# aitrailblazer/VectorRAGQuantization

Measured on AMD Instinct MI355X. Metric: queries/sec + recall@10 vs float32, d=1024 3-phase search at 1/2/4/8 GPUs, higher is better.
Workload: dtype u8+f64; 1 GPU; BASELINE config 4: CohereEnhancedVectorDB 3-phase search, row-sharded over N GPUs + RCCL all_gather of per-shard top-K, 100000000 x 1024 corpus, nq=1024 queries per step; corpus_rows=100000000, rows_per_gpu=100000000, nq=1024, k=10, binary_oversample=10, int8_oversample=3, parallelism=1 GPU

## Files before the change

### vectorragquantization_amd/csrc/hamming_mfma.hip

```cpp
#include <stdlib.h>

#include "mfma_common.h"
#include "mfma_fp4.h"
#include "mfma_hits.h"
#include "vrq_internal.h"
#include "vrq_scan.h"

namespace vrq {

constexpr int KS = 16;
constexpr int NG = 2 * KS;
constexpr int PKT = RT * 128;
constexpr int NPK = 4;
constexpr int NUB = 3;
constexpr int UBT = NG * 1024;
constexpr int GPW = (PKT / 1024) / MWAVES;
constexpr int BAHEAD = 3;
constexpr int NRING = BAHEAD < 4 ? 4 : 8;
#ifndef VRQ_K1M_NSR
#define VRQ_K1M_NSR 4
#endif
#ifndef VRQ_K1M_DMA_SHADOW
#define VRQ_K1M_DMA_SHADOW 1
#endif
template <int MB>
struct MfmaShape {
  static constexpr int QPW = 32 * MB;
  static constexpr int QPB = MWAVES * QPW;
  static constexpr int NSR = VRQ_K1M_NSR < MB ? VRQ_K1M_NSR : MB;
  static constexpr int SMEM =
      NPK * PKT + NUB * UBT + NUB * RT * 4 + MWAVES * QPW * 8 + MWAVES * (STG + 1) * 4 + MWAVES * MB * 128;
  static_assert(SMEM <= 160 * 1024, "LDS budget");
};
constexpr int kMbLarge = 4, kMbSmall = 2;
constexpr int kMbLargeMinQueries = 512;
constexpr int kRowsMaxQueries = 128;

__device__ __forceinline__ int pk_slot(int r, int c) { return r * 8 + (c ^ ((r >> 1) & 7)); }

constexpr int ENT_V_BIAS = 1025;


constexpr int k1m_pre(int g) { return ((g & 7) == 1 ? 1 : 0) + (g == 12 ? 2 : 0); }
constexpr int k1m_post(int g, int mb, int nsr, bool dense) {
  const int j = g & 15;
  return ((g & 7) == 6 ? 2 : 0) + (g == 28 ? 1 : 0) + (!dense && j >= 4 + mb + nsr && j < 4 + 2 * mb ? 4 : 0) +
         (!dense && g == 20 + mb ? 1 : 0) + (!dense && g == 24 + mb ? 1 : 0);
}
constexpr int k1m_wait(int gi, int mb, int nsr, bool dense) {
  const int g0 = gi - BAHEAD;
  int n = 1 + k1m_pre(gi);
  for (int g = g0 < 0 ? 0 : g0; g < gi; ++g) n += (g == g0 ? 0 : 1) + k1m_pre(g) + k1m_post(g, mb, nsr, dense);
  return n < 15 ? n : 15;
}

template <int MODE, int MB>
__global__ __launch_bounds__(MWAVES * 64, 1) void hamming_mfma_kernel(
    const uint8_t* __restrict__ codes, int64_t n, int64_t row_begin, const uint8_t* __restrict__ queries, int nq,
    const int32_t* __restrict__ tau, uint64_t* __restrict__ cand, int32_t* __restrict__ ccnt, int capc,
    int64_t chunk_rows, int64_t chunk_stride, int64_t tile_stride, int nchunks, int nqb,
    const int32_t* __restrict__ rerun,
    const int32_t* __restrict__ qbflag, uint16_t* __restrict__ dv, int64_t dv_stride) {
  constexpr bool DENSE = MODE == MFMA_SAMPLE;
  constexpr int QPW = MfmaShape<MB>::QPW, QPB = MfmaShape<MB>::QPB;
  constexpr int NSR = DENSE ? 0 : MfmaShape<MB>::NSR;
  __shared__ __attribute__((aligned(16))) uint8_t smem[MfmaShape<MB>::SMEM];
  uint8_t* pk = smem;
  uint8_t* ub = smem + NPK * PKT;
  int32_t* pcr = (int32_t*)(smem + NPK * PKT + NUB * UBT);
  const int w = __builtin_amdgcn_readfirstlane(threadIdx.x >> 6);
  int32_t* lcnt = pcr + NUB * RT + w * QPW;
  int32_t* tq = pcr + NUB * RT + MWAVES * QPW + w * QPW;
  int32_t* stg = pcr + NUB * RT + 2 * MWAVES * QPW + w * (STG + 1);

  const int l = lane_id();
  const int h = l >> 5, ri = l & 31;
  const int nb = gridDim.x, b = blockIdx.x;
  const int xcd = b & 7, slot = b >> 3, q8 = nb >> 3, r8 = nb & 7;
  const int L = (xcd < r8 ? xcd * (q8 + 1) : r8 * (q8 + 1) + (xcd - r8) * q8) + slot;
  const int chunk = L / nqb;
  const int qb = L - chunk * nqb;
  if (chunk >= nchunks) return;
  if (qbflag && qbflag[qb] == 0) return;
#ifdef VRQ_K1M_STAMPS
  const uint64_t st_start = __builtin_amdgcn_s_memrealtime();
#endif
  const int64_t row0 = row_begin + (int64_t)chunk * chunk_stride;
  const bool strided = tile_stride != RT;
  const int64_t row1 = strided ? n : (row0 + chunk_rows < n) ? row0 + chunk_rows : n;
  if (row0 >= row1) return;
  const int nrows = strided ? (int)chunk_rows : (int)(row1 - row0);
  const int ntiles = (nrows + RT - 1) / RT;

  static_assert(GPW == 2, "piece offsets derived for two pieces per wave");
  uint32_t doff0;
  {
    const int p = w * GPW * 64 + l;
    const int r = p >> 3, c = (p & 7) ^ ((r >> 1) & 7);
    doff0 = (uint32_t)(r * 128 + c * 16);
  }
  auto issue = [&](int t) __attribute__((always_inline)) {
    uint8_t* buf = pk + (t % NPK) * PKT;
    const int64_t tr0 = row0 + (int64_t)t * tile_stride;
    uint32_t d0 = doff0;
    asm volatile("" : "+v"(d0));
    const uint32_t doff[GPW] = {d0, (d0 + 1024u) ^ 64u};
    if (__builtin_expect(tr0 + RT <= row1, 1)) {
      const uint8_t* base = codes + tr0 * 128;
#pragma unroll
      for (int i = 0; i < GPW; ++i)
        __builtin_amdgcn_global_load_lds(base + doff[i], (__attribute__((address_space(3))) void*)(buf + (w * GPW + i) * 1024),
                                         16, 0, 0);
    } else {
#pragma unroll
      for (int i = 0; i < GPW; ++i) {
        int64_t row = tr0 + (doff[i] >> 7);
        row = row < row1 ? row : row1 - 1;
        __builtin_amdgcn_global_load_lds(codes + row * 128 + (doff[i] & 127),
                                         (__attribute__((address_space(3))) void*)(buf + (w * GPW + i) * 1024), 16, 0, 0);
      }
    }
  };
  auto issue_piece = [&](const uint8_t* base, uint32_t slot_off, auto I) __attribute__((always_inline)) {
    constexpr int i = decltype(I)::value;
    uint32_t d0 = doff0;
    asm volatile("" : "+v"(d0));
    const uint32_t d = i == 0 ? d0 : (d0 + 1024u) ^ 64u;
    __builtin_amdgcn_global_load_lds(base + d, (__attribute__((address_space(3))) void*)(pk + slot_off + (w * GPW + i) * 1024),
                                     16, 0, 0);
  };
  const uint32_t pk0 = lds_addr(pk), ub0 = lds_addr(ub), pcr0 = lds_addr(pcr);
  const uint32_t lc0 = lds_addr(lcnt), stg0 = lds_addr(stg);
  uint32_t usrc[4], udst[4];
#pragma unroll
  for (int u = 0; u < 4; ++u) {
    const int unit = 4 * w + u, nblk = unit >> 3, p = unit & 7;
    const int r = nblk * 32 + ri;
    usrc[u] = (uint32_t)(pk_slot(r, p) * 16 + h * 8);
    udst[u] = (uint32_t)(((nblk * KS + 2 * p) * 64 + l) * 16);
  }
  const int pr = 16 * w + (l >> 2), pc0 = 2 * (l & 3);
  const uint32_t psrc0 = (uint32_t)(pk_slot(pr, pc0) * 16), psrc1 = (uint32_t)(pk_slot(pr, pc0 + 1) * 16);
  auto unpack_write = [&](const v2i& v, int u, uint32_t ubuf) __attribute__((always_inline)) {
    lds_write128(ubuf + udst[u], unpack_row32((uint32_t)v.x));
    lds_write128(ubuf + udst[u] + 1024, unpack_row32((uint32_t)v.y));
  };
  auto rowpc_write = [&](const v4i& a, const v4i& c, uint32_t pbuf) __attribute__((always_inline)) {
    int pc = (__popc(a.x) + __popc(a.y) + __popc(a.z) + __popc(a.w)) +
             (__popc(c.x) + __popc(c.y) + __popc(c.z) + __popc(c.w));
    pc += __builtin_amdgcn_update_dpp(0, pc, 0xB1, 0xf, 0xf, false);
    pc += __builtin_amdgcn_update_dpp(0, pc, 0x4E, 0xf, 0xf, false);
    if ((l & 3) == 0) lds_write32(pbuf + (uint32_t)(pr * 4), pc);
  };

  for (int t = 0; t < NPK && t < ntiles; ++t) issue(t);

  const int qbase = qb * QPB + w * QPW;
  v4i A[MB][KS];
#pragma unroll
  for (int m = 0; m < MB; ++m) {
    const int q = qbase + 32 * m + ri;
    const bool qok = q < nq && (!rerun || rerun[q]);
    const uint4* qp = reinterpret_cast<const uint4*>(queries + (int64_t)(qok ? q : 0) * 128);
    int pc = 0;
#pragma unroll
    for (int c = 0; c < 8; ++c) {
      const uint4 v = qp[c];
      const uint32_t wd[4] = {qok ? v.x : 0u, qok ? v.y : 0u, qok ? v.z : 0u, qok ? v.w : 0u};
      pc += __popc(wd[0]) + __popc(wd[1]) + __popc(wd[2]) + __popc(wd[3]);
      A[m][2 * c] = unpack_query32(h ? wd[2] : wd[0]);
      A[m][2 * c + 1] = unpack_query32(h ? wd[3] : wd[1]);
    }
    if (h == 0) tq[32 * m + ri] = DENSE ? 0 : qok ? tau[q] - pc : -0x40000000;
  }
#pragma unroll
  for (int m = 0; m < MB; ++m)
#pragma unroll
    for (int s = 0; s < KS; ++s) asm volatile("" : "+a"(A[m][s]));
  float* sd = reinterpret_cast<float*>(pcr + NUB * RT + 2 * MWAVES * QPW + MWAVES * (STG + 1)) + w * MB * 32;
#pragma unroll
  for (int m = 0; m < MB; ++m)
    if (l < 32) {
      const int g = l & 15, hh = l >> 4;
      sd[m * 32 + l] = 0.5f * (float)tq[32 * m + (g & 3) + 8 * (g >> 2) + 4 * hh];
    }
  const uint32_t sd0 = lds_addr(sd) + (uint32_t)(h * 64);
  auto load_seed = [&](v16f& a, int m) __attribute__((always_inline)) {
    v4i p0, p1, p2, p3;
    lds_read128(p0, sd0 + (uint32_t)(m * 128));
    lds_read128(p1, sd0 + (uint32_t)(m * 128 + 16));
    lds_read128(p2, sd0 + (uint32_t)(m * 128 + 32));
    lds_read128(p3, sd0 + (uint32_t)(m * 128 + 48));
    const v16i x = __builtin_shufflevector(__builtin_shufflevector(p0, p1, 0, 1, 2, 3, 4, 5, 6, 7),
                                           __builtin_shufflevector(p2, p3, 0, 1, 2, 3, 4, 5, 6, 7), 0, 1, 2, 3, 4,
                                           5, 6, 7, 8, 9, 10, 11, 12, 13, 14, 15);
    a = __builtin_bit_cast(v16f, x);
  };
  for (int i = l; i < QPW; i += 64) lcnt[i] = 0;
  __syncthreads();
  auto wait_tiles = [&](int k) __attribute__((always_inline)) {
    if (k <= 0) wait_vm<0>();
    else if (k == 1) wait_vm<GPW>();
    else if (k == 2) wait_vm<2 * GPW>();
    else if (k == 3) wait_vm<3 * GPW>();
    else wait_vm<4 * GPW>();
  };
  static_assert(NPK - 2 <= 4, "wait_tiles covers up to 4 tiles in flight");
  const int nissued = ntiles < NPK ? ntiles : NPK;
  wait_tiles(nissued - 2);
  barrier_all();
  {
    v2i pv[8];
    v4i pa[2], pb[2];
#pragma unroll
    for (int t = 0; t < 2; ++t) {
#pragma unroll
      for (int u = 0; u < 4; ++u) lds_read64(pv[4 * t + u], pk0 + (uint32_t)(t * PKT) + usrc[u]);
      lds_read128(pa[t], pk0 + (uint32_t)(t * PKT) + psrc0);
      lds_read128(pb[t], pk0 + (uint32_t)(t * PKT) + psrc1);
    }
    asm volatile("s_waitcnt lgkmcnt(0)"
                 : "+v"(pv[0]), "+v"(pv[1]), "+v"(pv[2]), "+v"(pv[3]), "+v"(pv[4]), "+v"(pv[5]), "+v"(pv[6]),
                   "+v"(pv[7]), "+v"(pa[0]), "+v"(pa[1]), "+v"(pb[0]), "+v"(pb[1])::"memory");
#pragma unroll
    for (int t = 0; t < 2; ++t) {
#pragma unroll
      for (int u = 0; u < 4; ++u) unpack_write(pv[4 * t + u], u, ub0 + (uint32_t)(t * UBT));
      rowpc_write(pa[t], pb[t], pcr0 + (uint32_t)(t * RT * 4));
    }
  }
  wait_tiles(nissued - 3);
  wait_lgkm0();

  const int64_t qstride = (int64_t)nchunks * capc;
  uint64_t* const cbase = cand + ((int64_t)qbase * nchunks + chunk) * capc;
  int nst = 0;
  int fe = 0, fpos = 0, nfl = 0;
  auto fkey = [&](int e, int64_t base_row) __attribute__((always_inline)) {
    return ((uint64_t)(uint32_t)(e >> ENT_V_SHIFT) << KEY_ROW_BITS) | (uint64_t)(base_row + (e & 127));
  };
  auto store_flushed = [&](int t) __attribute__((always_inline)) {
    if (__builtin_expect(nfl != 0, 0)) {
      const int ql = (fe >> ENT_Q_SHIFT) & 127;
#ifndef VRQ_K1M_PROBE_NOSTORE
      if (l < nfl && fpos < capc) cbase[ql * qstride + fpos] = fkey(fe, row0 + (int64_t)(t - 2) * RT);
#endif
      nfl = 0;
    }
  };
  auto flush_from = [&](int i_begin, int64_t base_row) __attribute__((always_inline)) {
    int lf = l;
    asm volatile("" : "+v"(lf));
    if (nst > STG) {
      for (int i = lf; i < QPW; i += 64) lds_add32(lc0 + (uint32_t)(i * 4), capc + 1);
      nst = STG;
    }
    for (int i0 = i_begin; i0 < nst; i0 += 64) {
      const int i = i0 + lf;
      int e = 0, pos = 0;
      if (i < nst) lds_read32(e, stg0 + (uint32_t)(i * 4));
      asm volatile("s_waitcnt lgkmcnt(0)" : "+v"(e)::"memory");
      const int ql = (e >> ENT_Q_SHIFT) & 127;
      if (i < nst) lds_add_rtn32(pos, lc0 + (uint32_t)(ql * 4), 1);
      asm volatile("s_waitcnt lgkmcnt(0)" : "+v"(pos)::"memory");
      if (i < nst && pos < capc) cbase[ql * qstride + pos] = fkey(e, base_row);
    }
    nst = 0;
  };
  auto block_hits = [&](const v16f& a, int m, int pc, float hp, int rel7) __attribute__((always_inline)) {
#pragma unroll
    for (int g = 0; g < 16; ++g) {
      const uint64_t mask = __ballot(a[g] > hp);
      if (mask) {
        int lo = l;
        asm volatile("" : "+v"(lo));
        if ((mask >> lo) & 1) {
          const int below = __builtin_amdgcn_mbcnt_hi((uint32_t)(mask >> 32),
                                                      __builtin_amdgcn_mbcnt_lo((uint32_t)mask, 0));
          const int ql = 32 * m + (g & 3) + 8 * (g >> 2) + 4 * (lo >> 5);
          const int v = pc - (int)(2.0f * a[g]);
          const int pos = nst + below < STG ? nst + below : STG;
          lds_write32(stg0 + (uint32_t)(pos * 4), ((v + ENT_V_BIAS) << ENT_V_SHIFT) | (ql << ENT_Q_SHIFT) | (rel7 - ri + (lo & 31)));
        }
        nst += __popcll(mask);
      }
    }
  };
  auto block_hits_fast = [&](const v16f& a, int m, int pc, float hp, int rel7) __attribute__((always_inline)) {
    uint32_t m16 = 0, mmid = 0, mhi = 0;
#pragma unroll
    for (int g = 0; g < 7; ++g) m16 |= (a[g] > hp ? 1u : 0u) << g;
    asm volatile("" : "+v"(m16));
    VRQ_SCHED_FENCE();
#pragma unroll
    for (int g = 7; g < 14; ++g) mmid |= (a[g] > hp ? 1u : 0u) << (g - 7);
    asm volatile("" : "+v"(mmid));
    VRQ_SCHED_FENCE();
#pragma unroll
    for (int g = 14; g < 16; ++g) mhi |= (a[g] > hp ? 1u : 0u) << (g - 14);
    asm volatile("" : "+v"(mmid), "+v"(mhi));
    m16 |= (mmid << 7) | (mhi << 14);
#ifdef VRQ_K1M_PROBE_NOSLOW
    if (false) {
#else
    if (__ballot((m16 & (m16 - 1)) != 0)) {
#endif
      block_hits(a, m, pc, hp, rel7);
    } else {
      const uint64_t lanes = __ballot(m16 != 0);
      if (m16) {
        const v16i b = __builtin_bit_cast(v16i, a);
        const int x0 = max(max(b[0], b[1]), b[2]), x1 = max(max(b[3], b[4]), b[5]), x2 = max(max(b[6], b[7]), b[8]);
        const int x3 = max(max(b[9], b[10]), b[11]), x4 = max(max(b[12], b[13]), b[14]);
        const float mx = __int_as_float(max(max(max(x0, x1), x2), max(max(x3, x4), b[15])));
        const int below = __builtin_amdgcn_mbcnt_hi((uint32_t)(lanes >> 32),
                                                    __builtin_amdgcn_mbcnt_lo((uint32_t)lanes, 0));
        int lo = l;
        asm volatile("" : "+v"(lo));
        const int g = __builtin_ctz(m16);
        const int ql = 32 * m + (g & 3) + 8 * (g >> 2) + 4 * (lo >> 5);
        const int v = pc - (int)(2.0f * mx);
        const int pos = nst + below < STG ? nst + below : STG;
        lds_write32(stg0 + (uint32_t)(pos * 4), ((v + ENT_V_BIAS) << ENT_V_SHIFT) | (ql << ENT_Q_SHIFT) | (rel7 - ri + (lo & 31)));
      }
      nst += __popcll(lanes);
    }
  };
  auto row_pc = [&](int pcv, int lr) __attribute__((always_inline)) {
    return lr < nrows ? pcv : 0x40000000;
  };
  DenseMin<DENSE, MB, 1024> dmin;
  auto block_dense = [&](const v16f& a, int m, int pc, int lr) __attribute__((always_inline)) {
    dmin.fold(a, m, pc, lr < nrows);
  };

  v4i ring[NRING];
  const uint32_t bl0 = ub0 + (uint32_t)(l * 16);
  int pcvP = 0;
  int lmax = 0;
  uint64_t anyhit = 0;
  int hpb = 0;
  v16f acc[2][MB];
  v16f seedr[NSR > 0 ? NSR : 1];
  static_for<0, NSR>([&](auto M) {
    constexpr int m = decltype(M)::value;
    v4i p0, p1, p2, p3;
    lds_read128(p0, sd0 + (uint32_t)(m * 128));
    lds_read128(p1, sd0 + (uint32_t)(m * 128 + 16));
    lds_read128(p2, sd0 + (uint32_t)(m * 128 + 32));
    lds_read128(p3, sd0 + (uint32_t)(m * 128 + 48));
    asm volatile("s_waitcnt lgkmcnt(0)" : "+v"(p0), "+v"(p1), "+v"(p2), "+v"(p3)::"memory");
    const v16i x = __builtin_shufflevector(__builtin_shufflevector(p0, p1, 0, 1, 2, 3, 4, 5, 6, 7),
                                           __builtin_shufflevector(p2, p3, 0, 1, 2, 3, 4, 5, 6, 7), 0, 1, 2, 3, 4,
                                           5, 6, 7, 8, 9, 10, 11, 12, 13, 14, 15);
    seedr[m] = __builtin_bit_cast(v16f, x);
    acc[0][m] = acc[1][m] = seedr[m];
  });
  if constexpr (!DENSE)
    static_for<NSR, MB>([&](auto M) {
      constexpr int m = decltype(M)::value;
      load_seed(acc[0][m], m);
      load_seed(acc[1][m], m);
    });
  barrier_all();
#ifdef VRQ_K1M_STAMPS
  const uint64_t st_loop = __builtin_amdgcn_s_memrealtime();
#endif
  static_for<0, BAHEAD>([&](auto G) {
    constexpr int g = decltype(G)::value;
    lds_read128_imm<g * 1024>(ring[g], bl0);
  });
  __builtin_assume(ntiles > 0);
  const int nwhole = strided ? ntiles : nrows / RT;
  const int nsteady = nwhole > NPK ? nwhole - NPK : 0;
  int ru0 = 0, ru1 = 1, ru2 = 2;
  uint32_t pko = 0;
  const int64_t dstep = tile_stride * 128;
  const uint8_t* dsrc = codes + (row0 + (int64_t)NPK * tile_stride) * 128;
#ifdef VRQ_K1M_STAMPS
  uint32_t st_a = 0, st_b = 0, st_bsum = 0;
#endif
  for (int t = 0; t < ntiles; ++t) {
    store_flushed(t);
    const bool steady = t < nsteady;
    if (__builtin_expect(steady, 1)) {
      if constexpr (!VRQ_K1M_DMA_SHADOW) {
        issue_piece(dsrc, pko, std::integral_constant<int, 0>{});
        issue_piece(dsrc, pko, std::integral_constant<int, 1>{});
      }
    } else if (t + NPK < ntiles) {
      issue(t + NPK);
    }
    const uint32_t blt = bl0 + (uint32_t)(ru0 * UBT);
    const uint32_t bln = bl0 + (uint32_t)(ru1 * UBT);
    const uint32_t ubw = ub0 + (uint32_t)(ru2 * UBT);
    const uint32_t pks = pk0 + (pko ^ (uint32_t)(2 * PKT));
    static_assert(NPK == 4 && NUB == 3, "ring walks: slot of t + 2 by XOR, unpacked slots by rotation");
    int pcv[2];
    const uint32_t pcra = pcr0 + (uint32_t)((ru0 * RT + ri) * 4);
    lds_read32_imm<0>(pcv[0], pcra);
    lds_read32_imm<32 * 4>(pcv[1], pcra);
    v2i pv;
    v4i pa, pb;
    VRQ_SCHED_FENCE();
    static_for<0, NG>([&](auto GI) {
      constexpr int gi = decltype(GI)::value;
      constexpr int nbk = gi >> 4, s = gi & 15, j = gi & 15;
      if constexpr (gi + BAHEAD < NG)
        lds_read128_imm<(gi + BAHEAD) * 1024>(ring[(gi + BAHEAD) & (NRING - 1)], blt);
      else
        lds_read128_imm<(gi + BAHEAD - NG) * 1024>(ring[(gi + BAHEAD) & (NRING - 1)], bln);
      if constexpr ((gi & 7) == 1) lds_read64(pv, xor_add<16 * (gi >> 3)>(usrc[0], pks));
      if constexpr (gi == 12) {
        lds_read128(pa, xor_add<0>(psrc0, pks));
        lds_read128(pb, xor_add<16>(psrc0, pks));
      }
      asm volatile("s_waitcnt lgkmcnt(%7)"
                   : "+v"(ring[gi & (NRING - 1)]), "+v"(pv), "+v"(pcv[0]), "+v"(pcv[1]), "+v"(pa), "+v"(pb), "+v"(fe)
                   : "n"(k1m_wait(gi, MB, NSR, DENSE))
                   : "memory");
      constexpr bool TEST = !DENSE && j >= 2 && j < 2 + MB;
      constexpr int tm = TEST ? j - 2 : 0;
      constexpr bool UNPACK = (gi & 7) == 6;
      constexpr bool SEED = !DENSE && j >= 4 + MB + NSR && j < 4 + 2 * MB;
      constexpr int sm = SEED ? j - 4 - MB : 0;
      int e0 = 0, e1 = 0, e2 = 0, e3 = 0, e4 = 0, f0 = 0;
      uint32_t u0 = 0, u1 = 0, u2 = 0;
      int pc0 = 0, pc1 = 0;
      auto slot = [&](auto K) __attribute__((always_inline)) {
        constexpr int k = decltype(K)::value;
        const v16i bb = __builtin_bit_cast(v16i, acc[nbk ^ 1][tm]);
        if constexpr (TEST) {
          if constexpr (k == 0) {
            e0 = max(max(bb[0], bb[1]), bb[2]);
            e1 = max(max(bb[3], bb[4]), bb[5]);
            asm volatile("" ::"v"(e0), "v"(e1));
          } else if constexpr (k == 1) {
            e2 = max(max(bb[6], bb[7]), bb[8]);
            e3 = max(max(bb[9], bb[10]), bb[11]);
            asm volatile("" ::"v"(e2), "v"(e3));
          } else if constexpr (k == 2) {
            e4 = max(max(bb[12], bb[13]), bb[14]);
            f0 = max(max(e0, e1), e2);
            asm volatile("" ::"v"(e4), "v"(f0));
          } else {
            const int mx = max(max(e3, e4), f0);
            lmax = tm == 0 ? max(bb[15], mx) : max(max(lmax, bb[15]), mx);
            if constexpr (tm == MB - 1) anyhit = __ballot(lmax > hpb);
          }
        }
        if constexpr (!DENSE && j == 1 && k == 0) {
          const int pcr_ = nbk == 0 ? pcvP : pcv[0];
          const int lr = (nbk == 0 ? (t - 1) * RT + 32 : t * RT) + ri;
          hpb = (nbk == 0 && t == 0) ? 0x7fffffff : __float_as_int(0.5f * (float)row_pc(pcr_, lr));
          asm volatile("" : "+v"(hpb));
        }
        if constexpr (UNPACK) {
          constexpr int half = k >> 1;
          const uint32_t wv = (uint32_t)(half ? pv.y : pv.x);
          if constexpr ((k & 1) == 0) {
            u0 = wv & 0x11111111u;
            u1 = wv & 0x22222222u;
            u2 = wv & 0x44444444u;
            asm volatile("" ::"v"(u0), "v"(u1), "v"(u2));
          } else {
            v4i r;
            r.x = (int)u0;
            r.y = (int)u1;
            r.z = (int)u2;
            r.w = (int)((wv >> 1) & 0x44444444u);
            lds_write128_imm<(gi >> 3) * 2048 + half * 1024>(ubw + udst[0], r);
          }
        }
        if constexpr (gi == 28) {
          if constexpr (k == 0) {
            pc0 = __popc(pa.x) + __popc(pa.y) + __popc(pa.z) + __popc(pa.w);
            asm volatile("" ::"v"(pc0));
          } else if constexpr (k == 1) {
            pc1 = __popc(pb.x) + __popc(pb.y) + __popc(pb.z) + __popc(pb.w);
            asm volatile("" ::"v"(pc1));
          } else if constexpr (k == 2) {
            pc0 = pc0 + pc1;
            pc0 += __builtin_amdgcn_update_dpp(0, pc0, 0xB1, 0xf, 0xf, false);
            asm volatile("" ::"v"(pc0));
          } else {
            pc0 += __builtin_amdgcn_update_dpp(0, pc0, 0x4E, 0xf, 0xf, false);
            lds_write32(pcr0 + (uint32_t)(ru2 * RT * 4 + pr * 4), pc0);
          }
        }
        if constexpr (SEED) {
          v4i piece;
          lds_read128(piece, sd0 + (uint32_t)(sm * 128 + k * 16));
          v16i x = __builtin_bit_cast(v16i, acc[nbk ^ 1][sm]);
          x[4 * k] = piece.x;
          x[4 * k + 1] = piece.y;
          x[4 * k + 2] = piece.z;
          x[4 * k + 3] = piece.w;
          acc[nbk ^ 1][sm] = __builtin_bit_cast(v16f, x);
        }
        if constexpr (DENSE && j >= 2 && j < 2 + MB && k == 0) {
          if (nbk == 1 || t > 0) {
            const int pcr_ = nbk == 0 ? pcvP : pcv[0];
            const int lr = (nbk == 0 ? (t - 1) * RT + 32 : t * RT) + ri;
            block_dense(acc[nbk ^ 1][j - 2], j - 2, pcr_, lr);
          }
        }
        if constexpr (VRQ_K1M_DMA_SHADOW && gi == 0 && (k == 0 || k == 2)) {
          if (__builtin_expect(steady, 1)) issue_piece(dsrc, pko, std::integral_constant<int, k / 2>{});
        }
        if constexpr (gi == NG - 1) {
          if constexpr (k == 0) {
            const int r = ru0;
            ru0 = ru1;
            ru1 = ru2;
            ru2 = r;
            asm volatile("" : "+s"(ru0), "+s"(ru1), "+s"(ru2));
          } else if constexpr (k == 1) {
            pko = (pko + (uint32_t)PKT) & (uint32_t)(NPK * PKT - 1);
            asm volatile("" : "+s"(pko));
          } else if constexpr (k == 2) {
            dsrc += dstep;
            asm volatile("" : "+s"(dsrc));
          }
        }
        if constexpr (k == 3) {
          if constexpr (gi == 20 + MB && !DENSE) {
            lds_read32(fe, stg0 + (uint32_t)(l * 4));
            nfl = nst < 64 ? nst : 64;
          }
          if constexpr (gi == 24 + MB && !DENSE)
            lds_add_rtn32(fpos, lc0 + (uint32_t)(((fe >> ENT_Q_SHIFT) & 127) * 4), l < nfl ? 1 : 0);
          if constexpr (!DENSE && j == 3 + MB) {
            if (__builtin_expect(anyhit != 0, 0)) {
              const int pcr_ = nbk == 0 ? pcvP : pcv[0];
              const int lr = (nbk == 0 ? (t - 1) * RT + 32 : t * RT) + ri;
              const int pc = row_pc(pcr_, lr);
              const float hp = 0.5f * (float)pc;
              static_for<0, MB>([&](auto M) {
                constexpr int mm = decltype(M)::value;
#ifndef VRQ_K1M_PROBE_NOHITS
                if (any_above(acc[nbk ^ 1][mm], hp))
                  block_hits_fast(acc[nbk ^ 1][mm], mm, pc, hp, (nbk == 0 ? 32 : 64) + ri);
#endif
              });
            }
          }
        }
      };
      static_for<0, MB>([&](auto M) {
        constexpr int m = decltype(M)::value;
        if constexpr (s == 0 && m < NSR) {
          acc[nbk][m] = mfma_fp4(A[m][s], ring[gi & (NRING - 1)], seedr[m < NSR ? m : 0]);
        } else {
          if constexpr (s == 0 && !DENSE)
            asm volatile("" : "+v"(acc[nbk][m]));
          acc[nbk][m] = mfma_fp4(A[m][s], ring[gi & (NRING - 1)], (s == 0 && DENSE) ? v16f{} : acc[nbk][m]);
        }
        asm volatile("" : "+v"(acc[nbk][m]));
        VRQ_SCHED_FENCE();
#ifdef VRQ_K1M_STAMPS
        if constexpr (gi == 0 && m == 0) st_b = (uint32_t)__builtin_amdgcn_s_memtime();
#endif
        if constexpr (MB == 4) {
          slot(std::integral_constant<int, m>{});
        } else {
          slot(std::integral_constant<int, 2 * m>{});
          slot(std::integral_constant<int, 2 * m + 1>{});
        }
        VRQ_SCHED_FENCE();
      });
      VRQ_SCHED_FENCE();
    });
    pcvP = pcv[1];
#ifdef VRQ_K1M_STAMPS
    const uint32_t st_an = (uint32_t)__builtin_amdgcn_s_memtime();
#endif
    {
#ifndef VRQ_K1M_PROBE_NOVMWAIT
      if (__builtin_expect(steady, 1)) {
        wait_vm<GPW>();
      } else {
        const int last = t + NPK < ntiles ? t + NPK : ntiles - 1;
        wait_tiles(last - (t + 3));
      }
#endif
    }
    asm volatile("s_waitcnt lgkmcnt(0)" : "+v"(fpos), "+v"(fe)::"memory");
#ifdef VRQ_K1M_STAMPS
    if (t > 0) st_bsum += st_b - st_a;
    st_a = st_an;
#endif
    if (__builtin_expect(nst > 64, 0))
      flush_from(64, row0 + (int64_t)(t - 1) * RT);
    nst = 0;
#ifndef VRQ_K1M_PROBE_NOBARRIER
    barrier_all();
#endif
  }
  store_flushed(ntiles);
  if (ntiles > 0) {
    const int lr = (ntiles - 1) * RT + 32 + ri;
    const int pc = row_pc(pcvP, lr);
    const float hp = 0.5f * (float)pc;
    static_for<0, MB>([&](auto M) {
      constexpr int m = decltype(M)::value;
      if constexpr (DENSE)
        block_dense(acc[1][m], m, pcvP, lr);
      else
        if (any_above(acc[1][m], hp)) block_hits_fast(acc[1][m], m, pc, hp, 96 + ri);
    });
    if (nst) flush_from(0, row0 + (int64_t)(ntiles - 2) * RT);
  }
  wait_lgkm0();
#ifdef VRQ_K1M_STAMPS
  if (!DENSE && threadIdx.x == 0) {
    uint64_t* stp = reinterpret_cast<uint64_t*>(dv) + 8 * (int64_t)L;
    stp[0] = st_start;
    stp[1] = st_loop;
    stp[2] = __builtin_amdgcn_s_memrealtime();
    stp[3] = ((uint64_t)__builtin_amdgcn_s_getreg(63508) << 32) | (uint32_t)__builtin_amdgcn_s_getreg(63492);
    stp[4] = ((uint64_t)(uint32_t)(ntiles - 1) << 32) | st_bsum;
  }
#endif
  if constexpr (DENSE)
    dmin.out(dv, dv_stride, (int64_t)chunk * 32 + ri, qbase, h, nq);
  else {
    int lz = l;
    asm volatile("" : "+v"(lz));
    for (int i = lz; i < QPW; i += 64) {
      const int q = qbase + i;
      if (q < nq && (!rerun || rerun[q])) ccnt[(int64_t)q * nchunks + chunk] = lcnt[i];
    }
  }
}

constexpr double kSwapMaxPairs = 4294967296.0;
#ifndef VRQ_K1S_LARGE
#define VRQ_K1S_LARGE 0
#endif
#ifndef VRQ_K1S_RB4
#define VRQ_K1S_RB4 0
#endif

constexpr int SQPB = 512;
template <int SRB, int SNW>
struct SwapShape {
  static constexpr int SRS = SRB * 32;
  static constexpr int QBYTES = SQPB * 128;
  static constexpr int RBYTES = SRS * 128;
  static constexpr int SMEM = QBYTES + SNW * RBYTES + SQPB * 4  + SQPB * 4  +
                              SNW * (STG + 1) * 4 + SNW * SRB * 32 * 4 ;
  static_assert(SMEM <= 160 * 1024, "LDS budget");
  static_assert(SRS <= 128, "a staged entry keeps 7 bits of row in the row set");
  static_assert((SRB == 2 && SNW == 8) || (SRB == 4 && SNW == 4), "the two instances");
};
constexpr int SENT_V_SHIFT = 16, SENT_Q_SHIFT = 7;

template <int MODE, int SRB, int SNW>
__global__ __launch_bounds__(SNW * 64, 1) void hamming_mfma_swap_kernel(
    const uint8_t* __restrict__ codes, int64_t n, int64_t row_begin, const uint8_t* __restrict__ queries, int nq,
    const int32_t* __restrict__ tau, uint64_t* __restrict__ cand, int32_t* __restrict__ ccnt, int capc,
    int64_t chunk_rows, int64_t chunk_stride, int64_t tile_stride, int nchunks, int nqb,
    const int32_t* __restrict__ rerun, const int32_t* __restrict__ qbflag, uint16_t* __restrict__ dv,
    int64_t dv_stride) {
  static_assert(MODE == MFMA_MAIN || MODE == MFMA_RERUN, "thresholded passes only");
  using Sh = SwapShape<SRB, SNW>;
  constexpr int SRS = Sh::SRS;
#ifndef VRQ_K1S_SPREAD
#define VRQ_K1S_SPREAD 1
#endif
  constexpr bool SPREAD = SNW == 4 && VRQ_K1S_SPREAD;
  __shared__ __attribute__((aligned(16))) uint8_t smem[Sh::SMEM];
  const int w = __builtin_amdgcn_readfirstlane(threadIdx.x >> 6);
  uint8_t* qpk = smem;
  uint8_t* rst = smem + Sh::QBYTES + w * Sh::RBYTES;
  float* thr = reinterpret_cast<float*>(smem + Sh::QBYTES + SNW * Sh::RBYTES);
  int32_t* lcnt = reinterpret_cast<int32_t*>(thr + SQPB);
  int32_t* stg = lcnt + SQPB + w * (STG + 1);
  float* sdw = reinterpret_cast<float*>(lcnt + SQPB + SNW * (STG + 1)) + w * SRB * 32;
  const int l = lane_id();
  const int h = l >> 5, ri = l & 31;
  const int nb = gridDim.x, b = blockIdx.x;
  const int xcd = b & 7, slot = b >> 3, q8 = nb >> 3, r8 = nb & 7;
  const int L = (xcd < r8 ? xcd * (q8 + 1) : r8 * (q8 + 1) + (xcd - r8) * q8) + slot;
  const int chunk = L / nqb;
  const int qb = L - chunk * nqb;
  if (chunk >= nchunks) return;
  if (qbflag && qbflag[qb] == 0) return;
  const int64_t row0 = row_begin + (int64_t)chunk * chunk_stride;
  const int64_t row1 = (row0 + chunk_rows < n) ? row0 + chunk_rows : n;
  if (row0 >= row1) return;
  const int nrs = (int)((row1 - row0 + SRS - 1) / SRS);
  const int qbase = qb * SQPB;
  const int nqv = nq - qbase < SQPB ? nq - qbase : SQPB;
  const int nqblk = (((nqv + 31) >> 5) + 1) & ~1;

  for (int p = threadIdx.x; p < SQPB * 8; p += SNW * 64) {
    const int j = p >> 3, c = p & 7, q = qbase + j;
    const bool qok = q < nq && (!rerun || rerun[q]);
    uint4 v = make_uint4(0u, 0u, 0u, 0u);
    if (qok) v = reinterpret_cast<const uint4*>(queries + (int64_t)q * 128)[c];
    reinterpret_cast<uint4*>(qpk)[pk_slot(j, c)] = v;
  }
  for (int j = threadIdx.x; j < SQPB; j += SNW * 64) {
    const int q = qbase + j;
    const bool qok = q < nq && (!rerun || rerun[q]);
    int pc = 0;
    if (qok) {
      const uint4* qp = reinterpret_cast<const uint4*>(queries + (int64_t)q * 128);
#pragma unroll
      for (int c = 0; c < 8; ++c) {
        const uint4 v = qp[c];
        pc += __popc(v.x) + __popc(v.y) + __popc(v.z) + __popc(v.w);
      }
    }
    thr[j] = qok ? 1024.0f + 0.5f * (float)(pc - tau[q]) : 1e30f;
    lcnt[j] = 0;
  }

  const int dcol0 = ((l & 7) ^ ((l >> 4) & 7)) * 16, dcol1 = ((l & 7) ^ ((4 + (l >> 4)) & 7)) * 16;
  const int dlane0 = (l >> 3) * 128 + dcol0, dlane1 = (l >> 3) * 128 + dcol1;
  auto issue = [&](int rs) __attribute__((always_inline)) {
    const int64_t r0 = row0 + (int64_t)rs * SRS;
    if (r0 + SRS <= row1) {
      const uint8_t* base = codes + r0 * 128;
#pragma unroll
      for (int i = 0; i < SRS / 8; ++i) {
        const uint8_t* src = base + i * 1024 + ((i & 1) ? dlane1 : dlane0);
        uint8_t* dst = rst + i * 1024;
        __builtin_amdgcn_global_load_lds(src, (__attribute__((address_space(3))) void*)dst, 16, 0, 0);
      }
    } else {
#pragma unroll
      for (int i = 0; i < SRS / 8; ++i) {
        int64_t row = r0 + 8 * i + (l >> 3);
        row = row < row1 ? row : row1 - 1;
        const uint8_t* src = codes + row * 128 + ((i & 1) ? dcol1 : dcol0);
        uint8_t* dst = rst + i * 1024;
        __builtin_amdgcn_global_load_lds(src, (__attribute__((address_space(3))) void*)dst, 16, 0, 0);
      }
    }
  };
  if (w < nrs) issue(w);
  __syncthreads();

  const uint32_t q0 = lds_addr(qpk), rst0 = lds_addr(rst), thr0 = lds_addr(thr), lc0 = lds_addr(lcnt);
  const uint32_t stg0 = lds_addr(stg), sdw0 = lds_addr(sdw);
  const int64_t qstride = (int64_t)nchunks * capc;
  uint64_t* const cbase = cand + ((int64_t)qbase * nchunks + chunk) * capc;
  int nst = 0;
  int ovf_qb = 1 << 20;
  auto flush = [&](int64_t base_row) __attribute__((always_inline)) {
    if (nst > STG) {
      for (int i = ovf_qb * 32 + l; i < nqblk * 32; i += 64) lds_add32(lc0 + (uint32_t)(i * 4), capc + 1);
      nst = STG;
      ovf_qb = 1 << 20;
    }
    for (int i0 = 0; i0 < nst; i0 += 64) {
      const int i = i0 + l;
      int e = 0, pos = 0;
      if (i < nst) lds_read32(e, stg0 + (uint32_t)(i * 4));
      asm volatile("s_waitcnt lgkmcnt(0)" : "+v"(e)::"memory");
      const int ql = (e >> SENT_Q_SHIFT) & (SQPB - 1);
      if (i < nst) lds_add_rtn32(pos, lc0 + (uint32_t)(ql * 4), 1);
      asm volatile("s_waitcnt lgkmcnt(0)" : "+v"(pos)::"memory");
      if (i < nst && pos < capc)
        cbase[(int64_t)ql * qstride + pos] =
            ((uint64_t)(uint32_t)(e >> SENT_V_SHIFT) << KEY_ROW_BITS) | (uint64_t)(base_row + (e & 127));
    }
    nst = 0;
  };
  auto block_hits = [&](const v16f& a, int rb, float th, int qbp) __attribute__((always_inline)) {
    uint32_t m16 = 0;
#pragma unroll
    for (int g = 0; g < 16; ++g) m16 |= (a[g] > th ? 1u : 0u) << g;
    int lo = l;
    asm volatile("" : "+v"(lo));
    const int qrow = ((qbp * 32 + (lo & 31)) << SENT_Q_SHIFT) + 32 * rb + 4 * (lo >> 5);
    if (__ballot((m16 & (m16 - 1)) != 0)) {
#pragma unroll
      for (int g = 0; g < 16; ++g) {
        const uint64_t mask = __ballot((m16 >> g) & 1);
        if (mask) {
          if ((m16 >> g) & 1) {
            const int below = __builtin_amdgcn_mbcnt_hi((uint32_t)(mask >> 32),
                                                        __builtin_amdgcn_mbcnt_lo((uint32_t)mask, 0));
            const int v = (int)(2.0f * th - 2.0f * a[g]);
            const int pos = nst + below < STG ? nst + below : STG;
            lds_write32(stg0 + (uint32_t)(pos * 4), ((v + ENT_V_BIAS) << SENT_V_SHIFT) | (qrow + (g & 3) + 8 * (g >> 2)));
          }
          nst += __popcll(mask);
          if (nst > STG && qbp < ovf_qb) ovf_qb = qbp;
        }
      }
    } else {
      const uint64_t lanes = __ballot(m16 != 0);
      if (m16) {
        const v16i x = __builtin_bit_cast(v16i, a);
        const int x0 = max(max(x[0], x[1]), x[2]), x1 = max(max(x[3], x[4]), x[5]), x2 = max(max(x[6], x[7]), x[8]);
        const int x3 = max(max(x[9], x[10]), x[11]), x4 = max(max(x[12], x[13]), x[14]);
        const float mx = __int_as_float(max(max(max(x0, x1), x2), max(max(x3, x4), x[15])));
        const int below = __builtin_amdgcn_mbcnt_hi((uint32_t)(lanes >> 32),
                                                    __builtin_amdgcn_mbcnt_lo((uint32_t)lanes, 0));
        const int g = __builtin_ctz(m16);
        const int v = (int)(2.0f * th - 2.0f * mx);
        const int pos = nst + below < STG ? nst + below : STG;
        lds_write32(stg0 + (uint32_t)(pos * 4), ((v + ENT_V_BIAS) << SENT_V_SHIFT) | (qrow + (g & 3) + 8 * (g >> 2)));
      }
      nst += __popcll(lanes);
      if (nst > STG && qbp < ovf_qb) ovf_qb = qbp;
    }
  };

  const int nmine = w < nrs ? (nrs - w + SNW - 1) / SNW : 0;
  if (nmine > 0) {
    v4i A[SRB][KS];
    auto write_seed = [&](int rb, int pc, int64_t r0) __attribute__((always_inline)) {
      const float sv = r0 + 32 * rb + ri < row1 ? 1024.0f - 0.5f * (float)pc : -4096.0f;
      if (h == 0)
        lds_write32(sdw0 + (uint32_t)((rb * 32 + ((ri >> 2) & 1) * 16 + (ri & 3) + 4 * (ri >> 3)) * 4), __float_as_int(sv));
    };
    auto rebuild = [&](int64_t r0) __attribute__((always_inline)) {
      static_for<0, SRB>([&](auto RB) {
        constexpr int rb = decltype(RB)::value;
        const int r = 32 * rb + ri;
        v4i p[4];
#pragma unroll
        for (int i = 0; i < 4; ++i) lds_read128(p[i], rst0 + (uint32_t)(pk_slot(r, 4 * h + i) * 16));
        asm volatile("s_waitcnt lgkmcnt(0)" : "+v"(p[0]), "+v"(p[1]), "+v"(p[2]), "+v"(p[3])::"memory");
        int pc = 0;
#pragma unroll
        for (int s = 0; s < KS; ++s) {
          const uint32_t wd = (uint32_t)p[s >> 2][s & 3];
          pc += __popc(wd);
          A[rb][s] = unpack_query32(wd);
          asm volatile("" : "+a"(A[rb][s]));
        }
        pc += __shfl_xor(pc, 32, 64);
        write_seed(rb, pc, r0);
      });
    };
    auto read_seed = [&](int rb) __attribute__((always_inline)) {
      v4i p[4];
#pragma unroll
      for (int i = 0; i < 4; ++i) lds_read128(p[i], sdw0 + (uint32_t)(rb * 128 + h * 64 + i * 16));
      const v16i x = __builtin_shufflevector(__builtin_shufflevector(p[0], p[1], 0, 1, 2, 3, 4, 5, 6, 7),
                                             __builtin_shufflevector(p[2], p[3], 0, 1, 2, 3, 4, 5, 6, 7), 0, 1, 2, 3,
                                             4, 5, 6, 7, 8, 9, 10, 11, 12, 13, 14, 15);
      return __builtin_bit_cast(v16f, x);
    };
    auto read_seed_now = [&](int rb) __attribute__((always_inline)) {
      v4i p[4];
#pragma unroll
      for (int i = 0; i < 4; ++i) lds_read128(p[i], sdw0 + (uint32_t)(rb * 128 + h * 64 + i * 16));
      asm volatile("s_waitcnt lgkmcnt(0)" : "+v"(p[0]), "+v"(p[1]), "+v"(p[2]), "+v"(p[3])::"memory");
      const v16i x = __builtin_shufflevector(__builtin_shufflevector(p[0], p[1], 0, 1, 2, 3, 4, 5, 6, 7),
                                             __builtin_shufflevector(p[2], p[3], 0, 1, 2, 3, 4, 5, 6, 7), 0, 1, 2, 3,
                                             4, 5, 6, 7, 8, 9, 10, 11, 12, 13, 14, 15);
      return __builtin_bit_cast(v16f, x);
    };
    auto read_qblock = [&](v4i (&wq)[4], int& thb, int qbi) __attribute__((always_inline)) {
      const int j = qbi * 32 + ri;
#pragma unroll
      for (int i = 0; i < 4; ++i) lds_read128_inplace(wq[i], q0 + (uint32_t)(pk_slot(j, 4 * h + i) * 16));
      lds_read32_inplace(thb, thr0 + (uint32_t)(j * 4));
    };

    v16f acc[2][SRB];
    v4i wq[2][4] = {};
    int thb[2] = {};
    auto retire = [&](auto C) __attribute__((always_inline)) {
      constexpr int c = decltype(C)::value;
      (void)acc, (void)wq, (void)thb;
      if constexpr (SRB == 2)
        asm volatile("s_waitcnt lgkmcnt(0)"
                     : "+v"(acc[c][0]), "+v"(acc[c][1]), "+v"(wq[c][0]), "+v"(wq[c][1]), "+v"(wq[c][2]),
                       "+v"(wq[c][3]), "+v"(thb[c])::"memory");
      else
        asm volatile("s_waitcnt lgkmcnt(0)"
                     : "+v"(acc[c][0]), "+v"(acc[c][1]), "+v"(acc[c][2]), "+v"(acc[c][3]), "+v"(wq[c][0]),
                       "+v"(wq[c][1]), "+v"(wq[c][2]), "+v"(wq[c][3]), "+v"(thb[c])::"memory");
    };
    auto stage_read = [&](v4i (&sg)[SRB], int grp) __attribute__((always_inline)) {
      static_for<0, SRB>([&](auto RB) {
        constexpr int rb = decltype(RB)::value;
        lds_read128_inplace(sg[rb], rst0 + (uint32_t)(pk_slot(32 * rb + ri, 4 * h + grp) * 16));
      });
    };
    auto retire_sg = [&](v4i (&sg)[SRB]) __attribute__((always_inline)) {
      static_assert(!SPREAD || SRB == 4, "the wait names four row blocks' staging registers");
      if constexpr (SPREAD)
        asm volatile("s_waitcnt lgkmcnt(0)" : "+v"(sg[0]), "+v"(sg[1]), "+v"(sg[2]), "+v"(sg[3])::"memory");
    };

    wait_vm<0>();
    rebuild(row0 + (int64_t)w * SRS);
    if (nmine > 1) issue(w + SNW);
    static_for<0, SRB>([&](auto RB) { acc[0][RB] = read_seed(RB); });
    read_qblock(wq[0], thb[0], 0);
    retire(std::integral_constant<int, 0>{});

    bool have_prev = false;
    int prev_qb = 0;
    int kset = 0;
    int64_t set_base = row0 + (int64_t)w * SRS;
    int64_t stage_base = set_base;
    auto qblock = [&](auto PAR, auto SWC, int qbi) __attribute__((always_inline)) {
      constexpr int c = decltype(PAR)::value;
      constexpr bool SW = decltype(SWC)::value;
      retire(std::integral_constant<int, c>{});
      v4i sg[SRB] = {};
      int spc[SRB] = {};
      if constexpr (SW) {
        wait_vm<0>();
        stage_read(sg, 0);
      }
      static_for<0, KS>([&](auto S) {
        constexpr int s = decltype(S)::value;
        const v4i bq = unpack_row32((uint32_t)wq[c][s >> 2][s & 3]);
        static_for<0, SRB>([&](auto RB) {
          acc[c][RB] = mfma_fp4(A[RB][s], bq, acc[c][RB]);
          if constexpr (SW) asm volatile("" : "+v"(acc[c][RB]));
        });
        if constexpr (SW) VRQ_SCHED_FENCE();
        if constexpr (SW) {
          if constexpr ((s & 3) == 0) retire_sg(sg);
          static_for<0, SRB>([&](auto RB) {
            constexpr int rb = decltype(RB)::value;
            const uint32_t wd = (uint32_t)sg[rb][s & 3];
            spc[rb] += __popc(wd);
            A[rb][s] = unpack_query32(wd);
            asm volatile("" : "+a"(A[rb][s]));
          });
          if constexpr ((s & 3) == 3 && s < KS - 1) stage_read(sg, (s >> 2) + 1);
        }
        if constexpr (s == 1) {
          if (have_prev) {
            const float th = __int_as_float(thb[c ^ 1]);
            uint64_t hm[SRB], any = 0;
            static_for<0, SRB>([&](auto RB) {
              const v16i x = __builtin_bit_cast(v16i, acc[c ^ 1][RB]);
              const int x0 = max(max(x[0], x[1]), x[2]), x1 = max(max(x[3], x[4]), x[5]);
              const int x2 = max(max(x[6], x[7]), x[8]), x3 = max(max(x[9], x[10]), x[11]);
              const int x4 = max(max(x[12], x[13]), x[14]);
              hm[RB] = __ballot(max(max(max(x0, x1), x2), max(max(x3, x4), x[15])) > thb[c ^ 1]);
              any |= hm[RB];
            });
            if (any) {
              static_for<0, SRB>([&](auto RB) {
                if (hm[RB]) block_hits(acc[c ^ 1][RB], RB, th, prev_qb);
              });
            }
          }
        }
        if constexpr (s == 2) {
          if (qbi == 0) {
            if (have_prev && nst) flush(stage_base);
            stage_base = set_base;
          }
        }
        if constexpr (s == 3) {
          const int nxt = qbi + 1 < nqblk ? qbi + 1 : 0;
          if constexpr (!SW) static_for<0, SRB>([&](auto RB) { acc[c ^ 1][RB] = read_seed(RB); });
          read_qblock(wq[c ^ 1], thb[c ^ 1], nxt);
        }
      });
      if constexpr (SW) {
        const int64_t nb0 = row0 + (int64_t)(w + SNW * (kset + 1)) * SRS;
        static_for<0, SRB>([&](auto RB) {
          constexpr int rb = decltype(RB)::value;
          const int pc = spc[rb] + __shfl_xor(spc[rb], 32, 64);
          write_seed(rb, pc, nb0);
        });
        static_for<0, SRB>([&](auto RB) { acc[c ^ 1][RB] = read_seed_now(RB); });
        if (kset + 2 < nmine) issue(w + SNW * (kset + 2));
        set_base = nb0;
        ++kset;
      }
      have_prev = true;
      prev_qb = qbi;
    };

    using F = std::false_type;
    using T = std::true_type;
    using P0 = std::integral_constant<int, 0>;
    using P1 = std::integral_constant<int, 1>;
    for (int k = 0; k < nmine; ++k) {
      if constexpr (SPREAD) {
        for (int qp = 0; qp + 2 < nqblk; qp += 2) {
          qblock(P0{}, F{}, qp);
          qblock(P1{}, F{}, qp + 1);
        }
        qblock(P0{}, F{}, nqblk - 2);
        qblock(P1{}, T{}, nqblk - 1);
      } else {
        for (int qp = 0; qp < nqblk; qp += 2) {
          qblock(P0{}, F{}, qp);
          qblock(P1{}, F{}, qp + 1);
        }
      }
      if (!SPREAD && k + 1 < nmine) {
        wait_vm<0>();
        retire(P0{});
        set_base = row0 + (int64_t)(w + SNW * (k + 1)) * SRS;
        rebuild(set_base);
        if (k + 2 < nmine) issue(w + SNW * (k + 2));
        static_for<0, SRB>([&](auto RB) { acc[0][RB] = read_seed(RB); });
        retire(P0{});
      }
    }
    {
      retire(P0{});
      const float th = __int_as_float(thb[1]);
      static_for<0, SRB>([&](auto RB) {
        const v16i x = __builtin_bit_cast(v16i, acc[1][RB]);
        const int x0 = max(max(x[0], x[1]), x[2]), x1 = max(max(x[3], x[4]), x[5]);
        const int x2 = max(max(x[6], x[7]), x[8]), x3 = max(max(x[9], x[10]), x[11]);
        const int x4 = max(max(x[12], x[13]), x[14]);
        if (__ballot(max(max(max(x0, x1), x2), max(max(x3, x4), x[15])) > thb[1])) block_hits(acc[1][RB], RB, th, prev_qb);
      });
      if (nst) flush(stage_base);
    }
  }
  wait_lgkm0();
  __syncthreads();
  for (int j = threadIdx.x; j < SQPB; j += SNW * 64) {
    const int q = qbase + j;
    if (q < nq && (!rerun || rerun[q])) ccnt[(int64_t)q * nchunks + chunk] = lcnt[j];
  }
}

template <int MB>
struct RowsShape {
  static_assert(MB == 1 || MB == 4, "M-blocks per wave (MB = 2: hamming_mfma_rows_lean_kernel)");
  static constexpr int QPW = 32 * MB;
  static constexpr int OCC = MB == 1 ? 2 : 1;
  static constexpr int NPR = MB == 1 ? 2 : 3;
  static constexpr bool SEEDREG = MB <= 2;
  static constexpr int SMEM = MWAVES * (NPR * PKT + QPW * 8 + (STG + 1) * 4 + MB * 128);
  static_assert(SMEM * OCC <= 160 * 1024, "LDS budget");
};
constexpr int K1R_AUX = 2;

template <int MODE, int MB>
__global__ __launch_bounds__(MWAVES * 64, RowsShape<MB>::OCC) void hamming_mfma_rows_kernel(
    const uint8_t* __restrict__ codes, int64_t n, const uint8_t* __restrict__ queries, int nq,
    const int32_t* __restrict__ tau, uint64_t* __restrict__ cand, int32_t* __restrict__ ccnt, int capc,
    int64_t chunk_rows, int64_t chunk_stride, int64_t tile_stride, int nchunks, const int32_t* __restrict__ rerun,
    const int32_t* __restrict__ qbflag, uint16_t* __restrict__ dv, int64_t dv_stride) {
  constexpr bool DENSE = MODE == MFMA_SAMPLE;
  constexpr int QPW = RowsShape<MB>::QPW;
  constexpr int NPR = RowsShape<MB>::NPR;
  constexpr bool SEEDREG = RowsShape<MB>::SEEDREG;
  if (qbflag && qbflag[0] == 0) return;
  __shared__ __attribute__((aligned(16))) uint8_t smem[RowsShape<MB>::SMEM];
  const int w = __builtin_amdgcn_readfirstlane(threadIdx.x >> 6);
  uint8_t* pk = smem + w * (NPR * PKT);
  int32_t* wbase = reinterpret_cast<int32_t*>(smem + MWAVES * NPR * PKT);
  int32_t* lcnt = wbase + w * QPW;
  int32_t* tq = wbase + MWAVES * QPW + w * QPW;
  int32_t* stg = wbase + 2 * MWAVES * QPW + w * (STG + 1);
  float* sd = reinterpret_cast<float*>(wbase + 2 * MWAVES * QPW + MWAVES * (STG + 1)) + w * MB * 32;
  const int l = lane_id();
  const int h = l >> 5, ri = l & 31;
  const int nb = gridDim.x, b = blockIdx.x;
  const int xcd = b & 7, slot = b >> 3, q8 = nb >> 3, r8 = nb & 7;
  const int L = (xcd < r8 ? xcd * (q8 + 1) : r8 * (q8 + 1) + (xcd - r8) * q8) + slot;
  const int chunk = L * MWAVES + w;
  if (chunk >= nchunks) return;
  const int64_t row0 = (int64_t)chunk * chunk_stride;
  const bool strided = tile_stride != RT;
  const int64_t row1 = strided ? n : (row0 + chunk_rows < n) ? row0 + chunk_rows : n;
  if (row0 >= row1) return;
  const int nrows = strided ? (int)chunk_rows : (int)(row1 - row0);
  const int ntiles = (nrows + RT - 1) / RT;
  const int nblk = 2 * ntiles;

  uint32_t doff[8];
#pragma unroll
  for (int i = 0; i < 8; ++i) {
    const int p = i * 64 + l;
    const int r = p >> 3, c = (p & 7) ^ ((r >> 1) & 7);
    doff[i] = (uint32_t)(r * 128 + c * 16);
  }
  auto issue = [&](int t) __attribute__((always_inline)) {
    uint8_t* buf = pk + (t % NPR) * PKT;
    const int64_t tr0 = row0 + (int64_t)t * tile_stride;
    if (tr0 + RT <= row1) {
      const uint8_t* base = codes + tr0 * 128;
#pragma unroll
      for (int i = 0; i < 8; ++i) {
        const uint8_t* src = base + doff[i];
        uint8_t* dst = buf + i * 1024;
        __builtin_amdgcn_global_load_lds(src, (__attribute__((address_space(3))) void*)dst, 16, 0, K1R_AUX);
      }
    } else {
#pragma unroll
      for (int i = 0; i < 8; ++i) {
        int64_t row = tr0 + (doff[i] >> 7);
        row = row < row1 ? row : row1 - 1;
        const uint8_t* src = codes + row * 128 + (doff[i] & 127);
        uint8_t* dst = buf + i * 1024;
        __builtin_amdgcn_global_load_lds(src, (__attribute__((address_space(3))) void*)dst, 16, 0, 0);
      }
    }
  };
  for (int t = 0; t < NPR && t < ntiles; ++t) issue(t);

  v4i A[MB][KS];
#pragma unroll
  for (int m = 0; m < MB; ++m) {
    const int q = 32 * m + ri;
    const bool qok = q < nq && (!rerun || rerun[q]);
    const uint32_t* qp = reinterpret_cast<const uint32_t*>(queries + (int64_t)(qok ? q : 0) * 128);
    int pc = 0;
#pragma unroll
    for (int s = 0; s < KS; ++s) {
      const uint32_t wd = qok ? qp[16 * h + s] : 0u;
      pc += __popc(wd);
      A[m][s] = unpack_query32(wd);
    }
    pc += __shfl_xor(pc, 32, 64);
    if (h == 0) tq[q] = DENSE ? 0 : qok ? tau[q] - pc : -0x40000000;
  }
#pragma unroll
  for (int m = 0; m < MB; ++m)
#pragma unroll
    for (int s = 0; s < KS; ++s) asm volatile("" : "+a"(A[m][s]));
  for (int i = l; i < QPW; i += 64) lcnt[i] = 0;
#pragma unroll
  for (int m = 0; m < MB; ++m)
    if (l < 32) {
      const int g = l & 15, hh = l >> 4;
      sd[m * 32 + l] = 0.5f * (float)tq[32 * m + (g & 3) + 8 * (g >> 2) + 4 * hh];
    }
  const uint32_t sd0 = lds_addr(sd) + (uint32_t)(h * 64), stg0 = lds_addr(stg);
  const uint32_t lc0 = lds_addr(lcnt), pk0 = lds_addr(pk);
  auto load_seed = [&](v16f& a, int m, auto SYNC) __attribute__((always_inline)) {
    v4i p0, p1, p2, p3;
    lds_read128(p0, sd0 + (uint32_t)(m * 128));
    lds_read128(p1, sd0 + (uint32_t)(m * 128 + 16));
    lds_read128(p2, sd0 + (uint32_t)(m * 128 + 32));
    lds_read128(p3, sd0 + (uint32_t)(m * 128 + 48));
    if constexpr (decltype(SYNC)::value)
      asm volatile("s_waitcnt lgkmcnt(0)" : "+v"(p0), "+v"(p1), "+v"(p2), "+v"(p3)::"memory");
    const v16i x = __builtin_shufflevector(__builtin_shufflevector(p0, p1, 0, 1, 2, 3, 4, 5, 6, 7),
                                           __builtin_shufflevector(p2, p3, 0, 1, 2, 3, 4, 5, 6, 7), 0, 1, 2, 3, 4,
                                           5, 6, 7, 8, 9, 10, 11, 12, 13, 14, 15);
    a = __builtin_bit_cast(v16f, x);
  };
  v16f seedv[SEEDREG ? MB : 1];
  v16f acc[2][MB];
  if constexpr (!DENSE) {
#pragma unroll
    for (int m = 0; m < MB; ++m) load_seed(SEEDREG ? seedv[SEEDREG ? m : 0] : acc[0][m], m, std::true_type{});
  }
  auto read_rows = [&](v4i (&d)[4], int blk) __attribute__((always_inline)) {
    const int r = 32 * (blk & 1) + ri;
    const uint32_t base = pk0 + (uint32_t)(((blk >> 1) % NPR) * PKT);
#pragma unroll
    for (int i = 0; i < 4; ++i) lds_read128(d[i], base + (uint32_t)(pk_slot(r, 4 * h + i) * 16));
  };
  auto wait_tiles = [&](int k) __attribute__((always_inline)) {
    if (k <= 0) wait_vm<0>();
    else if (k == 1) wait_vm<8>();
    else wait_vm<16>();
  };
  static_assert(NPR - 1 <= 2, "wait_tiles covers up to 2 tiles in flight");
  wait_tiles((ntiles < NPR ? ntiles : NPR) - 1);
  v4i rb[2][4];
  read_rows(rb[0], 0);
  asm volatile("s_waitcnt lgkmcnt(0)" : "+v"(rb[0][0]), "+v"(rb[0][1]), "+v"(rb[0][2]), "+v"(rb[0][3])::"memory");

  const int64_t qstride = (int64_t)nchunks * capc;
  uint64_t* const cbase = cand + (int64_t)chunk * capc;
  HitStage<ENT_V_BIAS, QPW> hs{stg0, lc0, cbase, qstride, capc, l};

  DenseMin<DENSE, MB, 1024> dmin;
  int pcs = 0;
  int pprev = 0;
  int hpb = 0x7fffffff;
  uint64_t hitm[MB];
#pragma unroll
  for (int m = 0; m < MB; ++m) hitm[m] = 0;
  auto nblock = [&](auto PAR, int blk) __attribute__((always_inline)) {
    constexpr int par = decltype(PAR)::value;
    if (par == 1 && blk + 1 < nblk) {
      const int t1 = (blk + 1) >> 1;
      const int last = t1 + NPR - 1 < ntiles ? t1 + NPR - 1 : ntiles - 1;
      wait_tiles(last - t1);
    }
    const int lr = blk * 32 + ri;
    static_for<0, KS>([&](auto S) {
      constexpr int s = decltype(S)::value;
      const uint32_t wd = (uint32_t)rb[par][s >> 2][s & 3];
      const v4i bfrag = unpack_row32(wd);
      static_for<0, MB>([&](auto M) {
        constexpr int m = decltype(M)::value;
        if constexpr (s == 0 && DENSE)
          acc[par][m] = mfma_fp4(A[m][s], bfrag, v16f{});
        else if constexpr (s == 0 && SEEDREG)
          acc[par][m] = mfma_fp4(A[m][s], bfrag, seedv[SEEDREG ? m : 0]);
        else
          acc[par][m] = mfma_fp4(A[m][s], bfrag, acc[par][m]);
        asm volatile("" : "+v"(acc[par][m]));
      });
      VRQ_SCHED_FENCE();
      if constexpr (s == 0)
        pcs = __popc(wd);
      else
        pcs += __popc(wd);
      if constexpr (DENSE && s >= 1 && s < 1 + MB) {
        if (blk > 0) dmin.fold(acc[par ^ 1][s - 1], s - 1, pprev, lr - 32 < nrows);
      }
      if constexpr (!DENSE && s >= 1 && s < 1 + MB) {
        constexpr int m = s - 1;
        const v16i bb = __builtin_bit_cast(v16i, acc[par ^ 1][m]);
        const int x0 = max(max(bb[0], bb[1]), bb[2]), x1 = max(max(bb[3], bb[4]), bb[5]);
        const int x2 = max(max(bb[6], bb[7]), bb[8]), x3 = max(max(bb[9], bb[10]), bb[11]);
        const int x4 = max(max(bb[12], bb[13]), bb[14]);
        hitm[m] = __ballot(max(max(max(x0, x1), x2), max(max(x3, x4), bb[15])) > hpb);
      }
      if constexpr (!DENSE && s == MB + 1) {
        uint64_t any = hitm[0];
#pragma unroll
        for (int m = 1; m < MB; ++m) any |= hitm[m];
        if (any) {
          const int lrp = lr - 32;
          const int pc = lrp < nrows && blk > 0 ? pprev : 0x40000000;
          const float hp = 0.5f * (float)pc;
          static_for<0, MB>([&](auto M) {
            constexpr int mm = decltype(M)::value;
            if (hitm[mm]) hs.block_hits(acc[par ^ 1][mm], mm, pc, hp);
          });
          if (hs.nst) hs.flush_all(row0 + (int64_t)(blk - 1) * 32);
        }
      }
      if constexpr (!DENSE && !SEEDREG && s >= MB + 2 && s < 2 * MB + 2)
        load_seed(acc[par ^ 1][s - MB - 2], s - MB - 2, std::false_type{});
      if constexpr (s == 8)
        if (blk + 1 < nblk) read_rows(rb[par ^ 1], blk + 1);
      VRQ_SCHED_FENCE();
    });
    pprev = pcs + __shfl_xor(pcs, 32, 64);
    hpb = __float_as_int(0.5f * (float)(lr < nrows ? pprev : 0x40000000));
    if constexpr (!DENSE && !SEEDREG) {
      static_assert(MB == 4, "re-seeded instance");
      asm volatile("s_waitcnt lgkmcnt(0)"
                   : "+v"(rb[par ^ 1][0]), "+v"(rb[par ^ 1][1]), "+v"(rb[par ^ 1][2]), "+v"(rb[par ^ 1][3]),
                     "+v"(acc[par ^ 1][0]), "+v"(acc[par ^ 1][1]), "+v"(acc[par ^ 1][2]), "+v"(acc[par ^ 1][3])::"memory");
    } else {
      asm volatile("s_waitcnt lgkmcnt(0)"
                   : "+v"(rb[par ^ 1][0]), "+v"(rb[par ^ 1][1]), "+v"(rb[par ^ 1][2]), "+v"(rb[par ^ 1][3])::"memory");
    }
    if (par == 0 && (blk >> 1) + NPR < ntiles) issue((blk >> 1) + NPR);
  };
  for (int blk = 0; blk < nblk; blk += 2) {
    nblock(std::integral_constant<int, 0>{}, blk);
    nblock(std::integral_constant<int, 1>{}, blk + 1);
  }
  {
    constexpr int par = 1;
    const int lr = (nblk - 1) * 32 + ri;
    if constexpr (DENSE) {
      static_for<0, MB>([&](auto M) { dmin.fold(acc[par][decltype(M)::value], decltype(M)::value, pprev, lr < nrows); });
    } else {
      const int pc = lr < nrows ? pprev : 0x40000000;
      const float hp = 0.5f * (float)pc;
      static_for<0, MB>([&](auto M) {
        constexpr int mm = decltype(M)::value;
        if (any_above(acc[par][mm], hp)) hs.block_hits(acc[par][mm], mm, pc, hp);
      });
      if (hs.nst) hs.flush_all(row0 + (int64_t)(nblk - 1) * 32);
    }
  }
  wait_lgkm0();
  if constexpr (DENSE)
    dmin.out(dv, dv_stride, (int64_t)chunk * 32 + ri, 0, h, nq);
  else
    for (int i = l; i < QPW; i += 64)
      if (i < nq && (!rerun || rerun[i])) ccnt[(int64_t)i * nchunks + chunk] = lcnt[i];
}

template <int MB>
struct LeanShape {
  static_assert(MB == 2, "lean K1r: the MB = 2 instance");
  static constexpr int QPW = 32 * MB;
  static constexpr int OCC = 2;
  static constexpr int NPR = 2;
  static constexpr int SMEM = MWAVES * (NPR * PKT + QPW * 8 + (STG + 1) * 4 + MB * 128);
  static_assert(OCC * SMEM <= 160 * 1024, "LDS budget of two workgroups per CU");
};

template <int MODE, int MB>
__global__ __launch_bounds__(MWAVES * 64, LeanShape<MB>::OCC) void hamming_mfma_rows_lean_kernel(
    const uint8_t* __restrict__ codes, int64_t n, const uint8_t* __restrict__ queries, int nq,
    const int32_t* __restrict__ tau, uint64_t* __restrict__ cand, int32_t* __restrict__ ccnt, int capc,
    int64_t chunk_rows, int64_t chunk_stride, int64_t tile_stride, int nchunks, const int32_t* __restrict__ rerun,
    const int32_t* __restrict__ qbflag, uint16_t* __restrict__ dv, int64_t dv_stride) {
  constexpr bool DENSE = MODE == MFMA_SAMPLE;
  constexpr int QPW = LeanShape<MB>::QPW, NPR = LeanShape<MB>::NPR;
  if (qbflag && qbflag[0] == 0) return;
  __shared__ __attribute__((aligned(16))) uint8_t smem[LeanShape<MB>::SMEM];
  const int w = __builtin_amdgcn_readfirstlane(threadIdx.x >> 6);
  uint8_t* pk = smem + w * (NPR * PKT);
  int32_t* wbase = reinterpret_cast<int32_t*>(smem + MWAVES * NPR * PKT);
  int32_t* lcnt = wbase + w * QPW;
  int32_t* tq = wbase + MWAVES * QPW + w * QPW;
  int32_t* stg = wbase + 2 * MWAVES * QPW + w * (STG + 1);
  float* sd = reinterpret_cast<float*>(wbase + 2 * MWAVES * QPW + MWAVES * (STG + 1)) + w * MB * 32;
  const int l = lane_id();
  const int h = l >> 5, ri = l & 31;
  const int nb = gridDim.x, b = blockIdx.x;
  const int xcd = b & 7, slot = b >> 3, q8 = nb >> 3, r8 = nb & 7;
  const int L = (xcd < r8 ? xcd * (q8 + 1) : r8 * (q8 + 1) + (xcd - r8) * q8) + slot;
  const int chunk = L * MWAVES + w;
  if (chunk >= nchunks) return;
  const int64_t row0 = (int64_t)chunk * chunk_stride;
  const bool strided = tile_stride != RT;
  const int64_t row1 = strided ? n : (row0 + chunk_rows < n) ? row0 + chunk_rows : n;
  if (row0 >= row1) return;
  const int nrows = strided ? (int)chunk_rows : (int)(row1 - row0);
  const int ntiles = (nrows + RT - 1) / RT;
  const int nblk = 2 * ntiles;

  auto issue = [&](int t) __attribute__((always_inline)) {
    int lo_ = l;
    asm volatile("" : "+v"(lo_));
    const uint32_t lo0 = (uint32_t)((lo_ >> 3) * 128 + ((lo_ & 7) ^ (lo_ >> 4)) * 16);
    uint8_t* buf = pk + (t % NPR) * PKT;
    const int64_t tr0 = row0 + (int64_t)t * tile_stride;
    const bool whole = tr0 + RT <= row1;
#pragma unroll
    for (int i = 0; i < 8; ++i) {
      const uint32_t off = lo0 ^ (uint32_t)((i & 1) * 64);
      int64_t row = tr0 + 8 * i + (int64_t)(off >> 7);
      if (!whole) row = row < row1 ? row : row1 - 1;
      const uint8_t* src = codes + row * 128 + (off & 127);
      uint8_t* dst = buf + i * 1024;
      if (whole)
        __builtin_amdgcn_global_load_lds(src, (__attribute__((address_space(3))) void*)dst, 16, 0, K1R_AUX);
      else
        __builtin_amdgcn_global_load_lds(src, (__attribute__((address_space(3))) void*)dst, 16, 0, 0);
    }
  };
  for (int t = 0; t < NPR && t < ntiles; ++t) issue(t);

  v4i A[MB][KS];
#pragma unroll
  for (int m = 0; m < MB; ++m) {
    const int q = 32 * m + ri;
    const bool qok = q < nq && (!rerun || rerun[q]);
    const uint32_t* qp = reinterpret_cast<const uint32_t*>(queries + (int64_t)(qok ? q : 0) * 128);
    int pc = 0;
#pragma unroll
    for (int s = 0; s < KS; ++s) {
      const uint32_t wd = qok ? qp[16 * h + s] : 0u;
      pc += __popc(wd);
      A[m][s] = unpack_query32(wd);
    }
    pc += __shfl_xor(pc, 32, 64);
    if (h == 0) tq[q] = DENSE ? 0 : qok ? tau[q] - pc : -0x40000000;
  }
#pragma unroll
  for (int m = 0; m < MB; ++m)
#pragma unroll
    for (int s = 0; s < KS; ++s) asm volatile("" : "+a"(A[m][s]));
  for (int i = l; i < QPW; i += 64) lcnt[i] = 0;
#pragma unroll
  for (int m = 0; m < MB; ++m)
    if (l < 32) {
      const int g = l & 15, hh = l >> 4;
      sd[m * 32 + l] = 0.5f * (float)tq[32 * m + (g & 3) + 8 * (g >> 2) + 4 * hh];
    }
  const uint32_t sd0 = lds_addr(sd) + (uint32_t)(h * 64), stg0 = lds_addr(stg);
  const uint32_t lc0 = lds_addr(lcnt), pk0 = lds_addr(pk);
  v16f seedv[MB];
  if constexpr (!DENSE) {
#pragma unroll
    for (int m = 0; m < MB; ++m) {
      v4i p0, p1, p2, p3;
      lds_read128(p0, sd0 + (uint32_t)(m * 128));
      lds_read128(p1, sd0 + (uint32_t)(m * 128 + 16));
      lds_read128(p2, sd0 + (uint32_t)(m * 128 + 32));
      lds_read128(p3, sd0 + (uint32_t)(m * 128 + 48));
      asm volatile("s_waitcnt lgkmcnt(0)" : "+v"(p0), "+v"(p1), "+v"(p2), "+v"(p3)::"memory");
      const v16i x = __builtin_shufflevector(__builtin_shufflevector(p0, p1, 0, 1, 2, 3, 4, 5, 6, 7),
                                             __builtin_shufflevector(p2, p3, 0, 1, 2, 3, 4, 5, 6, 7), 0, 1, 2, 3,
                                             4, 5, 6, 7, 8, 9, 10, 11, 12, 13, 14, 15);
      seedv[m] = __builtin_bit_cast(v16f, x);
    }
  }
  auto read_quad = [&](v4i& d, int i, int blk) __attribute__((always_inline)) {
    const int r = 32 * (blk & 1) + ri;
    lds_read128_inplace(d, pk0 + (uint32_t)(((blk >> 1) % NPR) * PKT) + (uint32_t)(pk_slot(r, 4 * h + i) * 16));
  };
  auto wait_tiles = [&](int k) __attribute__((always_inline)) {
    if (k <= 0) wait_vm<0>();
    else wait_vm<8>();
  };
  static_assert(NPR - 1 <= 1, "wait_tiles covers one tile in flight");
  wait_tiles((ntiles < NPR ? ntiles : NPR) - 1);
  v4i rb[4];
#pragma unroll
  for (int i = 0; i < 4; ++i) read_quad(rb[i], i, 0);
  asm volatile("s_waitcnt lgkmcnt(0)" : "+v"(rb[0]), "+v"(rb[1]), "+v"(rb[2]), "+v"(rb[3])::"memory");

  const int64_t qstride = (int64_t)nchunks * capc;
  uint64_t* const cbase = cand + (int64_t)chunk * capc;
  HitStage<ENT_V_BIAS, QPW> hs{stg0, lc0, cbase, qstride, capc, l};
  DenseMin<DENSE, MB, 1024> dmin;
  v16f acc[MB];
  for (int blk = 0; blk < nblk; ++blk) {
    if ((blk & 1) && blk + 1 < nblk) {
      const int t1 = (blk + 1) >> 1;
      const int last = t1 + NPR - 1 < ntiles ? t1 + NPR - 1 : ntiles - 1;
      wait_tiles(last - t1);
    }
    const int nx = blk + 1 < nblk ? blk + 1 : blk;
    int pcs = 0;
    static_for<0, KS>([&](auto S) {
      constexpr int s = decltype(S)::value;
      const uint32_t wd = (uint32_t)rb[s >> 2][s & 3];
#ifdef VRQ_K1R_PROBE_NOUNPACK
      const v4i bfrag = {(int)wd, (int)wd, (int)wd, (int)wd};
#else
      const v4i bfrag = unpack_row32(wd);
#endif
      static_for<0, MB>([&](auto M) {
        constexpr int m = decltype(M)::value;
        if constexpr (s == 0 && DENSE)
          acc[m] = mfma_fp4(A[m][s], bfrag, v16f{});
        else if constexpr (s == 0)
          acc[m] = mfma_fp4(A[m][s], bfrag, seedv[m]);
        else
          acc[m] = mfma_fp4(A[m][s], bfrag, acc[m]);
        asm volatile("" : "+v"(acc[m]));
      });
      VRQ_SCHED_FENCE();
      pcs += __popc(wd);
      if constexpr ((s & 3) == 3) read_quad(rb[s >> 2], s >> 2, nx);
      VRQ_SCHED_FENCE();
    });
    const auto pp = __builtin_amdgcn_permlane32_swap((uint32_t)pcs, (uint32_t)pcs, false, false);
    const int prow = (int)(pp[0] + pp[1]);
    const int lr = blk * 32 + ri;
    if constexpr (DENSE) {
      static_for<0, MB>([&](auto M) { dmin.fold(acc[decltype(M)::value], decltype(M)::value, prow, lr < nrows); });
    } else {
      const int pc = lr < nrows ? prow : 0x40000000;
      const float hp = 0.5f * (float)pc;
      const int hpb = __float_as_int(hp);
      uint64_t hitm[MB];
      uint64_t any = 0;
      static_for<0, MB>([&](auto M) {
        constexpr int m = decltype(M)::value;
        const v16i bb = __builtin_bit_cast(v16i, acc[m]);
        const int x0 = max(max(bb[0], bb[1]), bb[2]), x1 = max(max(bb[3], bb[4]), bb[5]);
        const int x2 = max(max(bb[6], bb[7]), bb[8]), x3 = max(max(bb[9], bb[10]), bb[11]);
        const int x4 = max(max(bb[12], bb[13]), bb[14]);
        hitm[m] = __ballot(max(max(max(x0, x1), x2), max(max(x3, x4), bb[15])) > hpb);
        any |= hitm[m];
      });
      if (any) {
        static_for<0, MB>([&](auto M) {
          constexpr int m = decltype(M)::value;
          if (hitm[m]) hs.block_hits(acc[m], m, pc, hp);
        });
        if (hs.nst) hs.flush_all(row0 + (int64_t)blk * 32);
      }
    }
    asm volatile("s_waitcnt lgkmcnt(0)" : "+v"(rb[0]), "+v"(rb[1]), "+v"(rb[2]), "+v"(rb[3])::"memory");
    if (!(blk & 1) && (blk >> 1) + NPR < ntiles) issue((blk >> 1) + NPR);
  }
  wait_lgkm0();
  if constexpr (DENSE)
    dmin.out(dv, dv_stride, (int64_t)chunk * 32 + ri, 0, h, nq);
  else
    for (int i = l; i < QPW; i += 64)
      if (i < nq && (!rerun || rerun[i])) ccnt[(int64_t)i * nchunks + chunk] = lcnt[i];
}

int mfma_plan(int64_t n, int nq, int K, MfmaPlan* p) {
  if (nq < 1 || K < 1 || K > kMfmaMaxK) return VRQ_EUNSUPPORTED;
  const int em = tuning_int("VRQ_MFMA_MB", 0);
  p->mb = (em == 2 || em == 4) ? em : nq >= kMbLargeMinQueries ? kMbLarge : kMbSmall;
  p->qpb = p->mb == kMbLarge ? MfmaShape<kMbLarge>::QPB : MfmaShape<kMbSmall>::QPB;
  p->nqb = (nq + p->qpb - 1) / p->qpb;
  static_assert(SQPB == MfmaShape<kMbLarge>::QPB, "K1s serves K1m's MB = 4 query blocks");
  {
    const bool short_pass = (double)n * (double)nq <= kSwapMaxPairs;
    p->swap = p->mb != kMbLarge ? 0 : short_pass ? (VRQ_K1S_RB4 ? 2 : 1) : (VRQ_K1S_LARGE ? 2 : 0);
  }
  p->rows = nq <= kRowsMaxQueries && tuning_int("VRQ_MFMA_ROWS", 1) != 0;
  int rows_occ = 1;
  if (p->rows) {
    p->swap = 0;
    p->mb = nq <= 32 ? 1 : nq <= 64 ? 2 : 4;
    p->qpb = kRowsMaxQueries;
    p->nqb = 1;
    rows_occ = p->mb == 1 ? RowsShape<1>::OCC : p->mb == 2 ? LeanShape<2>::OCC : RowsShape<4>::OCC;
  }
  p->nqb_s = (nq + MfmaShape<kMbSmall>::QPB - 1) / MfmaShape<kMbSmall>::QPB;
  const int64_t ev = tuning_int("VRQ_SAMPLE_DIV", 0);
  const int64_t div = ev >= 2 ? ev : kMfmaSampleDiv;
  int64_t S = n / div;
  if (S > kMfmaMaxSample) S = kMfmaMaxSample;
  if (S < kMfmaMinSample) S = kMfmaMinSample;
  int64_t tiles = S / RT > 0 ? S / RT : 1;
  if (tiles > n / RT) tiles = n / RT;
  p->rows_sample = p->rows && p->mb <= 2;
  int64_t nsc = p->rows_sample ? 256 * MWAVES * rows_occ : 256 / p->nqb_s;
  if (nsc < 8) nsc = 8;
  if (nsc > tiles) nsc = tiles;
  const int64_t T = tiles / nsc;
  tiles = nsc * T;
  const int64_t ts = tiles > 1 ? (n - RT) / (tiles - 1) : RT;
  p->sample_chunk_rows = T * RT;
  p->sample_chunks = (int)nsc;
  p->sample_stride = T * ts;
  p->sample_tile_stride = ts;
  p->sample = tiles * RT;
  p->dvcols = nsc * 32;
  int64_t want = p->rows ? 256 * MWAVES * rows_occ : 256 / p->nqb;
  if (want < 1) want = 1;
  int64_t cr = (n + want - 1) / want;
  cr = (cr + RT - 1) / RT * RT;
  if (cr < RT) cr = RT;
  p->chunk_rows = cr;
  p->nchunks = (int)((n + cr - 1) / cr);
  mfma_plan_lists(p, n, nq, K);
  return VRQ_OK;
}

bool mfma_use(int64_t n, int nq, int K, int flags) {
  if (flags & VRQ_SEARCH_SCAN_VALU) return false;
  const bool ok = K <= kMfmaMaxK && n >= kMfmaMinRows;
  if (flags & VRQ_SEARCH_SCAN_MFMA) return ok;
  return ok && nq >= kMfmaMinQueries;
}

int mfma_scan_launch(const MfmaPlan& p, const uint8_t* codes, int64_t n, const uint8_t* q, int nq, int K,
                     uint8_t* ws, hipStream_t s, int flags) {
  constexpr int ALL = VRQ_SCAN_STAGE_PREFIX | VRQ_SCAN_STAGE_MATRIX | VRQ_SCAN_STAGE_RECHECK | VRQ_SCAN_STAGE_SUFFIX;
  const int st = (flags & ALL) ? (flags & ALL) : ALL;
  const MfmaWorkspace w(p, ws, nq);
  const bool sampled = p.j < K;
  const int32_t* none = nullptr;
  auto pass = [&](auto kswap2, auto kswap4, auto kern4, auto kern2, int grid, const int32_t* tau, uint64_t* cd,
                  int32_t* cc, int64_t crows, int64_t cstride, int nch, const int32_t* rr, const int32_t* qf,
                  uint16_t* d, int64_t dstride) {
    if (p.swap == 1)
      hipLaunchKernelGGL(kswap2, dim3(grid), dim3(8 * 64), 0, s, codes, n, (int64_t)0, q, nq, tau, cd, cc, p.capc,
                         crows, cstride, (int64_t)RT, nch, p.nqb, rr, qf, d, dstride);
    else if (p.swap == 2)
      hipLaunchKernelGGL(kswap4, dim3(grid), dim3(4 * 64), 0, s, codes, n, (int64_t)0, q, nq, tau, cd, cc, p.capc,
                         crows, cstride, (int64_t)RT, nch, p.nqb, rr, qf, d, dstride);
    else if (p.mb == kMbLarge)
      hipLaunchKernelGGL(kern4, dim3(grid), dim3(MWAVES * 64), 0, s, codes, n, (int64_t)0, q, nq, tau, cd, cc, p.capc,
                         crows, cstride, (int64_t)RT, nch, p.nqb, rr, qf, d, dstride);
    else
      hipLaunchKernelGGL(kern2, dim3(grid), dim3(MWAVES * 64), 0, s, codes, n, (int64_t)0, q, nq, tau, cd, cc, p.capc,
                         crows, cstride, (int64_t)RT, nch, p.nqb, rr, qf, d, dstride);
  };
  auto rows_pass = [&](auto k1, auto k2, auto k4, const int32_t* tau, const int32_t* rr, const int32_t* qf,
                       int nch, int64_t crows, int64_t cstride, int64_t tstride, uint16_t* d, int64_t dstride) {
    const dim3 g((unsigned)((nch + MWAVES - 1) / MWAVES)), blk(MWAVES * 64);
    if (p.mb == 1)
      hipLaunchKernelGGL(k1, g, blk, 0, s, codes, n, q, nq, tau, w.cand, w.ccnt, p.capc, crows, cstride, tstride, nch, rr,
                         qf, d, dstride);
    else if (p.mb == 2)
      hipLaunchKernelGGL(k2, g, blk, 0, s, codes, n, q, nq, tau, w.cand, w.ccnt, p.capc, crows, cstride, tstride, nch, rr,
                         qf, d, dstride);
    else
      hipLaunchKernelGGL(k4, g, blk, 0, s, codes, n, q, nq, tau, w.cand, w.ccnt, p.capc, crows, cstride, tstride, nch, rr,
                         qf, d, dstride);
  };
  if ((st & VRQ_SCAN_STAGE_PREFIX) && p.rows_sample) {
    if (p.mb > 2) return VRQ_EUNSUPPORTED;
    rows_pass(hamming_mfma_rows_kernel<MFMA_SAMPLE, 1>, hamming_mfma_rows_lean_kernel<MFMA_SAMPLE, 2>,
              hamming_mfma_rows_kernel<MFMA_SAMPLE, 1>, none, none, none, p.sample_chunks, p.sample_chunk_rows,
              p.sample_stride, p.sample_tile_stride, w.dv, p.dvcols);
    VRQ_LAUNCH_CHECK();
    const int rc = mfma_sample_select_launch(p, w, q, 128, nq, K, s);
    if (rc != VRQ_OK) return rc;
  } else if (st & VRQ_SCAN_STAGE_PREFIX) {
    hipLaunchKernelGGL((hamming_mfma_kernel<MFMA_SAMPLE, kMbSmall>), dim3(p.sample_chunks * p.nqb_s), dim3(MWAVES * 64),
                       0, s, codes, n, (int64_t)0, q, nq, none, (uint64_t*)nullptr, (int32_t*)nullptr, 0,
                       p.sample_chunk_rows, p.sample_stride, p.sample_tile_stride, p.sample_chunks, p.nqb_s, none,
                       none, w.dv, p.dvcols);
    VRQ_LAUNCH_CHECK();
    const int rc = mfma_sample_select_launch(p, w, q, 128, nq, K, s);
    if (rc != VRQ_OK) return rc;
  }
  if ((st & VRQ_SCAN_STAGE_MATRIX) && p.rows) {
    rows_pass(hamming_mfma_rows_kernel<MFMA_MAIN, 1>, hamming_mfma_rows_lean_kernel<MFMA_MAIN, 2>,
              hamming_mfma_rows_kernel<MFMA_MAIN, 4>, (const int32_t*)(sampled ? w.tau_s : w.tau_p), none, none,
              p.nchunks, p.chunk_rows, p.chunk_rows, (int64_t)RT, (uint16_t*)nullptr, (int64_t)0);
    VRQ_LAUNCH_CHECK();
  } else if (st & VRQ_SCAN_STAGE_MATRIX) {
#ifdef VRQ_K1M_STAMPS
    uint16_t* mdv = w.dv;
#else
    uint16_t* mdv = nullptr;
#endif
    pass(hamming_mfma_swap_kernel<MFMA_MAIN, 2, 8>, hamming_mfma_swap_kernel<MFMA_MAIN, 4, 4>,
         hamming_mfma_kernel<MFMA_MAIN, kMbLarge>,
         hamming_mfma_kernel<MFMA_MAIN, kMbSmall>, p.nchunks * p.nqb,
         (const int32_t*)(sampled ? w.tau_s : w.tau_p), w.cand, w.ccnt, p.chunk_rows, p.chunk_rows, p.nchunks, none, none,
         mdv, (int64_t)0);
    VRQ_LAUNCH_CHECK();
  }
  if ((st & VRQ_SCAN_STAGE_RECHECK) && sampled) {
    const int rc = mfma_sample_check_launch(p, w, nq, K, s);
    if (rc != VRQ_OK) return rc;
    if (p.rows)
      rows_pass(hamming_mfma_rows_kernel<MFMA_RERUN, 1>, hamming_mfma_rows_lean_kernel<MFMA_RERUN, 2>,
                hamming_mfma_rows_kernel<MFMA_RERUN, 4>, (const int32_t*)w.tau_p, (const int32_t*)w.rerun,
                (const int32_t*)w.qbflag, p.nchunks, p.chunk_rows, p.chunk_rows, (int64_t)RT, (uint16_t*)nullptr,
                (int64_t)0);
    else
      pass(hamming_mfma_swap_kernel<MFMA_RERUN, 2, 8>, hamming_mfma_swap_kernel<MFMA_RERUN, 4, 4>,
           hamming_mfma_kernel<MFMA_RERUN, kMbLarge>,
           hamming_mfma_kernel<MFMA_RERUN, kMbSmall>, p.nchunks * p.nqb,
           (const int32_t*)w.tau_p, w.cand, w.ccnt, p.chunk_rows, p.chunk_rows, p.nchunks, (const int32_t*)w.rerun,
           (const int32_t*)w.qbflag, (uint16_t*)nullptr, (int64_t)0);
    VRQ_LAUNCH_CHECK();
  }
  if (st & VRQ_SCAN_STAGE_SUFFIX) return mfma_suffix_launch(p, w, codes, n, 128, q, nq, K, s);
  return VRQ_OK;
}

}
```

### vectorragquantization_amd/csrc/mfma_threshold.hip

```cpp
#include <type_traits>

#include "vrq_internal.h"
#include "vrq_scan.h"

namespace vrq {

template <int CB>
struct ThrCode {
  static constexpr int DIM = 8 * CB;
  static constexpr int QW = CB / 4;
  static constexpr int NB = 2 * DIM + 1;
  static constexpr int KEY_BIAS = DIM + 1;
  static constexpr int HB = 2 * DIM + 2;
};

template <int CB>
__global__ __launch_bounds__(256) void sample_select_kernel(const uint16_t* __restrict__ dv, int64_t S,
                                                            const uint8_t* __restrict__ queries, int K, int j,
                                                            int32_t* __restrict__ tau_s, int32_t* __restrict__ tau_p,
                                                            int32_t* __restrict__ rerun, int32_t* __restrict__ qbflag,
                                                            int nqb) {
  constexpr int DIM = ThrCode<CB>::DIM, NB = ThrCode<CB>::NB;
  __shared__ uint32_t hist[NB + 3];
  __shared__ int pcq;
  const int qi = blockIdx.x, tid = threadIdx.x;
  if (qi == 0 && qbflag)
    for (int i = tid; i < nqb; i += 256) qbflag[i] = 0;
  for (int i = tid; i < NB; i += 256) hist[i] = 0;
  if (tid == 0) pcq = 0;
  __syncthreads();
  if (tid < ThrCode<CB>::QW)
    atomicAdd(&pcq, __popc(reinterpret_cast<const uint32_t*>(queries + (int64_t)qi * CB)[tid]));
  const uint16_t* d = dv + (int64_t)qi * S;
  const int64_t S8 = S & ~int64_t(7);
  constexpr int U = 8;
  auto add8 = [&](const uint4& w) {
    const uint32_t x[4] = {w.x, w.y, w.z, w.w};
#pragma unroll
    for (int k = 0; k < 4; ++k) {
      const uint32_t lo = x[k] & 0xffff, hi = x[k] >> 16;
      if (lo < (uint32_t)NB) atomicAdd(&hist[lo], 1u);
      if (hi < (uint32_t)NB) atomicAdd(&hist[hi], 1u);
    }
  };
  int64_t i = (int64_t)tid * 8;
  for (; i + (U - 1) * 256 * 8 < S8; i += U * 256 * 8) {
    uint4 w[U];
#pragma unroll
    for (int u = 0; u < U; ++u) w[u] = *reinterpret_cast<const uint4*>(d + i + u * 256 * 8);
#pragma unroll
    for (int u = 0; u < U; ++u) add8(w[u]);
  }
  for (; i < S8; i += 256 * 8) add8(*reinterpret_cast<const uint4*>(d + i));
  for (int64_t i = S8 + tid; i < S; i += 256)
    if (d[i] < NB) atomicAdd(&hist[d[i]], 1u);
  __syncthreads();
  if (tid < 64) {
    constexpr int BPL = (NB + 63) / 64;
    int loc = 0;
    for (int i = 0; i < BPL; ++i) {
      const int b = tid * BPL + i;
      if (b < NB) loc += (int)hist[b];
    }
    int inc = loc;
    for (int o = 1; o < 64; o <<= 1) {
      const int y = __shfl_up(inc, o, 64);
      if (tid >= o) inc += y;
    }
    int cum = inc - loc, rk = NB, rj = NB;
    for (int i = 0; i < BPL; ++i) {
      const int b = tid * BPL + i;
      if (b < NB) {
        const int hh = (int)hist[b];
        if (cum < K && cum + hh >= K) rk = b;
        if (cum < j && cum + hh >= j) rj = b;
        cum += hh;
      }
    }
    for (int o = 32; o > 0; o >>= 1) {
      rk = min(rk, __shfl_xor(rk, o, 64));
      rj = min(rj, __shfl_xor(rj, o, 64));
    }
    if (tid == 0) {
      const int dk = rk < NB ? rk - DIM + pcq : DIM;
      const int dj = rj < NB ? rj - DIM + pcq : DIM;
      tau_p[qi] = dk + 1;
      tau_s[qi] = (j < K ? dj : dk) + 1;
      rerun[qi] = 0;
    }
  }
}

__global__ __launch_bounds__(256) void sample_check_kernel(const int32_t* __restrict__ ccnt, int nchunks, int K,
                                                           int nq, int32_t* __restrict__ rerun,
                                                           int32_t* __restrict__ qbflag, int qpb) {
  const int q = blockIdx.x * 4 + (threadIdx.x >> 6), l = lane_id();
  if (q >= nq) return;
  int64_t c = 0;
  for (int i = l; i < nchunks; i += 64) c += ccnt[(int64_t)q * nchunks + i];
  c = wave_sum_i64(c);
  const bool fail = c < K;
  if (l == 0) {
    rerun[q] = fail ? 1 : 0;
    if (fail) atomicOr(&qbflag[q / qpb], 1);
  }
}

constexpr int SUF_THREADS = 256;
constexpr int SUF_CAP = 4096;
constexpr int SUF_MAX_CHUNKS = 2048;
static_assert(kMfmaMaxK <= SUF_THREADS, "the in-LDS filter needs K <= SUF_THREADS");

template <int CB>
struct SufShared {
  static constexpr int HB = ThrCode<CB>::HB;
  static constexpr int HW = (HB > SUF_MAX_CHUNKS + 1 ? HB : SUF_MAX_CHUNKS + 1) + 2;
  uint32_t hist[HW];
  uint64_t buf[SUF_CAP];
  uint32_t qw[ThrCode<CB>::QW];
  int32_t misc[8];
  int32_t scan[SUF_THREADS / WAVE];
};

template <int CB>
__device__ __forceinline__ int row_dist(const uint8_t* __restrict__ codes, int64_t r, const uint32_t (&qw)[CB / 4]) {
  const uint4* p = reinterpret_cast<const uint4*>(codes + r * CB);
  int d = 0;
#pragma unroll
  for (int c = 0; c < CB / 16; ++c) {
    const uint4 v = p[c];
    d += __popc(v.x ^ qw[4 * c]) + __popc(v.y ^ qw[4 * c + 1]) + __popc(v.z ^ qw[4 * c + 2]) +
         __popc(v.w ^ qw[4 * c + 3]);
  }
  return d;
}

__device__ inline int suf_excl_scan(int v, int* tot, int32_t* scratch) {
  const int l = lane_id(), w = threadIdx.x / WAVE;
  int x = v;
#pragma unroll
  for (int o = 1; o < WAVE; o <<= 1) {
    const int y = __shfl_up(x, o, WAVE);
    if (l >= o) x += y;
  }
  __syncthreads();
  if (l == WAVE - 1) scratch[w] = x;
  __syncthreads();
  int base = 0, all = 0;
  for (int i = 0; i < SUF_THREADS / WAVE; ++i) {
    const int s = scratch[i];
    if (i < w) base += s;
    all += s;
  }
  __syncthreads();
  *tot = all;
  return base + x - v;
}

template <int CB>
__device__ int suffix_rescan(const uint8_t* __restrict__ codes, int64_t n, int K, SufShared<CB>& sh) {
  constexpr int DIM = ThrCode<CB>::DIM, QW = ThrCode<CB>::QW;
  const int tid = threadIdx.x;
  for (int i = tid; i < DIM + 1; i += SUF_THREADS) sh.hist[i] = 0;
  __syncthreads();
  uint32_t qw[QW];
#pragma unroll
  for (int i = 0; i < QW; ++i) qw[i] = sh.qw[i];
  for (int64_t r = tid; r < n; r += SUF_THREADS) atomicAdd(&sh.hist[row_dist<CB>(codes, r, qw)], 1u);
  __syncthreads();
  if (tid == 0) {
    int cum = 0, T = DIM + 1, clt = 0;
    for (int d = 0; d < DIM + 1; ++d) {
      if (cum + (int)sh.hist[d] >= K) {
        T = d;
        clt = cum;
        break;
      }
      cum += (int)sh.hist[d];
    }
    if (T == DIM + 1) clt = cum;
    sh.misc[0] = T;
    sh.misc[1] = clt;
    sh.misc[2] = 0;
    sh.misc[3] = 0;
  }
  __syncthreads();
  const int T = sh.misc[0], clt = sh.misc[1];
  const int R = K - clt;
  for (int64_t base = 0; base < n; base += SUF_THREADS) {
    const int64_t r = base + tid;
    const int d = r < n ? row_dist<CB>(codes, r, qw) : 0x7fffffff;
    if (d < T) {
      const int pos = atomicAdd(&sh.misc[2], 1);
      sh.buf[pos] = ((uint64_t)(uint32_t)d << KEY_ROW_BITS) | (uint64_t)r;
    }
    const int eq = (d == T) ? 1 : 0;
    if (__syncthreads_or(eq)) {
      int tot;
      const int pre = suf_excl_scan(eq, &tot, sh.scan);
      const int rank = sh.misc[3] + pre;
      if (eq && rank < R) sh.buf[clt + rank] = ((uint64_t)(uint32_t)d << KEY_ROW_BITS) | (uint64_t)r;
      __syncthreads();
      if (tid == 0) sh.misc[3] += tot;
      __syncthreads();
    }
  }
  __syncthreads();
  const int taken = sh.misc[3] < R ? sh.misc[3] : R;
  return clt + (taken > 0 ? taken : 0);
}

template <int CB>
__global__ __launch_bounds__(SUF_THREADS) void suffix_topk_kernel(
    const uint8_t* __restrict__ codes, int64_t n, const uint8_t* __restrict__ queries,
    const uint64_t* __restrict__ cand, const int32_t* __restrict__ ccnt, int nchunks, int capc, int K,
    const int32_t* __restrict__ tau_main, const int32_t* __restrict__ tau_p, const int32_t* __restrict__ rerun,
    uint64_t* __restrict__ out) {
  using Sh = SufShared<CB>;
  constexpr int HB = Sh::HB;
  __shared__ Sh sh;
  const int qi = blockIdx.x, tid = threadIdx.x;
  if (tid < ThrCode<CB>::QW) sh.qw[tid] = reinterpret_cast<const uint32_t*>(queries + (int64_t)qi * CB)[tid];
  if (tid < 8) sh.misc[tid] = 0;
  __syncthreads();
  const int32_t* cq = ccnt + (int64_t)qi * nchunks;
  const uint64_t* Cq = cand + (int64_t)qi * nchunks * capc;
  auto vbin = [](uint64_t key) {
    const uint32_t f = (uint32_t)(key >> KEY_ROW_BITS);
    return f < (uint32_t)HB ? f : (uint32_t)(HB - 1);
  };
  const int CPT = (nchunks + SUF_THREADS - 1) / SUF_THREADS;
  int mine = 0, over = 0;
  for (int j = 0; j < CPT; ++j) {
    const int c = tid * CPT + j;
    if (c < nchunks) {
      const int v = cq[c];
      over |= v > capc;
      mine += v < capc ? v : capc;
    }
  }
  int total;
  int off = suf_excl_scan(mine, &total, sh.scan);
  const bool overflow = __syncthreads_or(over) != 0;
  const int tauq = (rerun && rerun[qi]) ? tau_p[qi] : tau_main[qi];
  const int64_t dfix = (int64_t)tauq - ThrCode<CB>::KEY_BIAS;
  int m = -1;
  bool real_dist = false;
  if (!overflow && total <= SUF_CAP && nchunks < Sh::HW) {
    int32_t* coff = reinterpret_cast<int32_t*>(sh.hist);
    for (int j = 0; j < CPT; ++j) {
      const int c = tid * CPT + j;
      if (c < nchunks) {
        const int v = cq[c];
        coff[c] = off;
        off += v < capc ? v : capc;
      }
    }
    if (tid == 0) coff[nchunks] = total;
    __syncthreads();
    for (int e = tid; e < total; e += SUF_THREADS) {
      int lo = 0, hi = nchunks;
      while (hi - lo > 1) {
        const int mid = (lo + hi) >> 1;
        if (coff[mid] <= e) lo = mid; else hi = mid;
      }
      sh.buf[e] = Cq[(int64_t)lo * capc + (e - coff[lo])];
    }
    m = total;
  } else if (!overflow) {
    for (int i = tid; i < HB; i += SUF_THREADS) sh.hist[i] = 0;
    __syncthreads();
    for (int c = 0; c < nchunks; ++c) {
      const int v = cq[c];
      for (int i = tid; i < v; i += SUF_THREADS) atomicAdd(&sh.hist[vbin(Cq[(int64_t)c * capc + i])], 1u);
    }
    __syncthreads();
    if (tid == 0) {
      int cum = 0, T = HB - 1;
      for (int d = 0; d < HB; ++d) {
        cum += (int)sh.hist[d];
        if (cum >= K) {
          T = d;
          break;
        }
      }
      sh.misc[5] = T;
      sh.misc[6] = cum;
      sh.misc[7] = 0;
    }
    __syncthreads();
    if (sh.misc[6] <= SUF_CAP) {
      const uint32_t T = (uint32_t)sh.misc[5];
      for (int c = 0; c < nchunks; ++c) {
        const int v = cq[c];
        for (int i = tid; i < v; i += SUF_THREADS) {
          const uint64_t key = Cq[(int64_t)c * capc + i];
          if (vbin(key) <= T) sh.buf[atomicAdd(&sh.misc[7], 1)] = key;
        }
      }
      __syncthreads();
      m = sh.misc[7];
    }
  }
  __syncthreads();
  if (m < 0) {
    m = suffix_rescan<CB>(codes, n, K, sh);
    real_dist = true;
  }
  __syncthreads();
  if (!real_dist && m > SUF_THREADS) {
    for (int i = tid; i < HB; i += SUF_THREADS) sh.hist[i] = 0;
    __syncthreads();
    for (int i = tid; i < m; i += SUF_THREADS) atomicAdd(&sh.hist[vbin(sh.buf[i])], 1u);
    __syncthreads();
    {
      constexpr int BPT = (HB + SUF_THREADS - 1) / SUF_THREADS;
      int loc = 0;
      for (int b = 0; b < BPT; ++b) {
        const int d = tid * BPT + b;
        if (d < HB) loc += (int)sh.hist[d];
      }
      int tot;
      int cum = suf_excl_scan(loc, &tot, sh.scan);
      for (int b = 0; b < BPT; ++b) {
        const int d = tid * BPT + b;
        if (d >= HB) break;
        const int h = (int)sh.hist[d];
        if (cum < K && cum + h >= K) sh.misc[5] = d;
        cum += h;
      }
      if (tid == 0) sh.misc[7] = 0;
    }
    __syncthreads();
    const uint32_t T = (uint32_t)sh.misc[5];
    constexpr int KPT = SUF_CAP / SUF_THREADS;
    uint64_t kk[KPT];
#pragma unroll
    for (int j = 0; j < KPT; ++j) kk[j] = tid + j * SUF_THREADS < m ? sh.buf[tid + j * SUF_THREADS] : KEY_NONE;
    __syncthreads();
#pragma unroll
    for (int j = 0; j < KPT; ++j)
      if (kk[j] != KEY_NONE && vbin(kk[j]) <= T) sh.buf[atomicAdd(&sh.misc[7], 1)] = kk[j];
    __syncthreads();
    m = sh.misc[7];
  }
  if (m <= SUF_THREADS) {
    const uint64_t ki = tid < m ? sh.buf[tid] : KEY_NONE;
    if (tid < 4) sh.buf[m + tid] = KEY_NONE;
    __syncthreads();
    int rank = 0;
    if (tid < m) {
      for (int j = 0; j < m; j += 4) {
        const uint64_t a = sh.buf[j], b = sh.buf[j + 1], c = sh.buf[j + 2], d = sh.buf[j + 3];
        rank += (a < ki ? 1 : 0) + (b < ki ? 1 : 0) + (c < ki ? 1 : 0) + (d < ki ? 1 : 0);
      }
    }
    __syncthreads();
    if (tid < m) sh.buf[rank] = ki;
    __syncthreads();
  } else {
    const int np2 = next_pow2(m);
    for (int i = m + tid; i < np2; i += SUF_THREADS) sh.buf[i] = KEY_NONE;
    __syncthreads();
    block_bitonic_sort_u64(sh.buf, np2);
  }
  uint64_t* o = out + (int64_t)qi * K;
  const uint64_t ROWM = (1ull << KEY_ROW_BITS) - 1;
  for (int i = tid; i < K; i += SUF_THREADS) {
    uint64_t key = KEY_NONE;
    if (i < m) {
      key = sh.buf[i];
      if (!real_dist) key = ((uint64_t)((int64_t)(key >> KEY_ROW_BITS) + dfix) << KEY_ROW_BITS) | (key & ROWM);
    }
    o[i] = key;
  }
}


template <class F>
static int for_cb(int cb, F&& f) {
  switch (cb) {
    case 32: return f(std::integral_constant<int, 32>{});
    case 48: return f(std::integral_constant<int, 48>{});
    case 64: return f(std::integral_constant<int, 64>{});
    case 96: return f(std::integral_constant<int, 96>{});
    case 128: return f(std::integral_constant<int, 128>{});
    case 192: return f(std::integral_constant<int, 192>{});
    case 256: return f(std::integral_constant<int, 256>{});
    default: return VRQ_EUNSUPPORTED;
  }
}

int mfma_sample_order(double lam, int K) {
  double term = __builtin_exp(-lam), cdf = 0.0;
  for (int j = 1; j < K; ++j) {
    cdf += term;
    if (1.0 - cdf <= 1e-6) return j;
    term *= lam / j;
  }
  return K;
}

void mfma_plan_lists(MfmaPlan* p, int64_t n, int nq, int K) {
  const int64_t expect = (K * p->chunk_rows + p->sample - 1) / p->sample;
  int capc = 64;
  while (capc < 4 * expect && capc < 4096) capc <<= 1;
  p->capc = capc;
  p->j = mfma_sample_order((double)K * (double)p->sample / (double)n, K);
  auto al = [](size_t x) { return (x + 255) & ~size_t(255); };
  p->off_suffix = al((size_t)nq * p->dvcols * sizeof(uint16_t));
  p->off_cand = p->off_suffix + al((size_t)nq * K * sizeof(uint64_t));
  p->off_cnt = p->off_cand + al((size_t)nq * p->nchunks * p->capc * sizeof(uint64_t));
  p->off_tau = p->off_cnt + al((size_t)nq * p->nchunks * sizeof(int32_t));
  p->bytes = p->off_tau + 3 * al((size_t)nq * sizeof(int32_t)) + (size_t)p->nqb * sizeof(int32_t);
}

int mfma_sample_select_launch(const MfmaPlan& p, const MfmaWorkspace& w, const uint8_t* q, int cb, int nq, int K,
                              hipStream_t s) {
  return for_cb(cb, [&](auto CBC) -> int {
    hipLaunchKernelGGL(sample_select_kernel<decltype(CBC)::value>, dim3(nq), dim3(256), 0, s, (const uint16_t*)w.dv,
                       p.dvcols, q, K, p.j, w.tau_s, w.tau_p, w.rerun, w.qbflag, p.nqb);
    VRQ_LAUNCH_CHECK();
    return VRQ_OK;
  });
}

int mfma_sample_check_launch(const MfmaPlan& p, const MfmaWorkspace& w, int nq, int K, hipStream_t s) {
  hipLaunchKernelGGL(sample_check_kernel, dim3((nq + 3) / 4), dim3(256), 0, s, (const int32_t*)w.ccnt, p.nchunks, K, nq,
                     w.rerun, w.qbflag, p.qpb);
  VRQ_LAUNCH_CHECK();
  return VRQ_OK;
}

int mfma_suffix_launch(const MfmaPlan& p, const MfmaWorkspace& w, const uint8_t* codes, int64_t n, int cb,
                       const uint8_t* q, int nq, int K, hipStream_t s) {
  const bool sampled = p.j < K;
  return for_cb(cb, [&](auto CBC) -> int {
    hipLaunchKernelGGL(suffix_topk_kernel<decltype(CBC)::value>, dim3(nq), dim3(SUF_THREADS), 0, s, codes, n, q,
                       (const uint64_t*)w.cand, (const int32_t*)w.ccnt, p.nchunks, p.capc, K,
                       (const int32_t*)(sampled ? w.tau_s : w.tau_p), (const int32_t*)w.tau_p,
                       (const int32_t*)(sampled ? w.rerun : nullptr), w.suffix);
    VRQ_LAUNCH_CHECK();
    return VRQ_OK;
  });
}

}
```

### vectorragquantization_amd/csrc/vrq_scan.h

```cpp
#pragma once
#include <hip/hip_runtime.h>
#include <stddef.h>
#include <stdint.h>

#include "../../include/vrq.h"

namespace vrq {

constexpr int64_t kTargetWaves = 4096;
constexpr int64_t kMinChunkRows = 4096;

struct ScanPlan {
  int cap;
  int qg;
  int wpg;
  int nqg;
  int64_t chunk_rows;
  int nchunks;
  size_t list_bytes;
};

int scan_plan(int64_t n, int cb, int nq, int K, ScanPlan* p);
int scan_launch(const ScanPlan& p, const uint8_t* codes, int64_t n, int cb, const uint8_t* q, int nq, int K,
                uint64_t* lists, hipStream_t s);

bool dim_code_bytes_supported(int cb);
int dim_scan_queries_per_wave(int cb);
int dim_scan_launch(const ScanPlan& p, const uint8_t* codes, int64_t n, int cb, const uint8_t* q, int nq, int K,
                    uint64_t* lists, hipStream_t s);

constexpr int kMfmaMaxK = 128;
#ifndef VRQ_MIN_SAMPLE
#define VRQ_MIN_SAMPLE 65536
#endif
constexpr int64_t kMfmaMinSample = VRQ_MIN_SAMPLE;
constexpr int64_t kMfmaMaxSample = 1 << 20;
constexpr int64_t kMfmaMinRows = 65536;
constexpr int kMfmaMinQueries = 1;
constexpr int64_t kMfmaSampleDiv = 32;

struct MfmaPlan {
  int64_t sample;
  int64_t dvcols;
  int64_t sample_chunk_rows;
  int64_t sample_stride;
  int64_t sample_tile_stride;
  int sample_chunks;
  int j;
  int capc;
  int rows;
  int swap;
  int rows_sample;
  int mb;
  int qpb;
  int nqb;
  int nqb_s;
  int64_t chunk_rows;
  int nchunks;
  size_t off_suffix, off_cand, off_cnt, off_tau, bytes;
};

int mfma_plan(int64_t n, int nq, int K, MfmaPlan* p);
bool mfma_use(int64_t n, int nq, int K, int flags);
int mfma_scan_launch(const MfmaPlan& p, const uint8_t* codes, int64_t n, const uint8_t* q, int nq, int K,
                     uint8_t* ws, hipStream_t s, int flags);

int mfma_sample_order(double lam, int K);
void mfma_plan_lists(MfmaPlan* p, int64_t n, int nq, int K);
struct MfmaWorkspace {
  uint16_t* dv;
  uint64_t *suffix, *cand;
  int32_t *ccnt, *tau_s, *tau_p, *rerun, *qbflag;
  MfmaWorkspace(const MfmaPlan& p, uint8_t* ws, int nq) {
    const size_t qa = ((size_t)nq * sizeof(int32_t) + 255) & ~size_t(255);
    dv = (uint16_t*)ws;
    suffix = (uint64_t*)(ws + p.off_suffix);
    cand = (uint64_t*)(ws + p.off_cand);
    ccnt = (int32_t*)(ws + p.off_cnt);
    tau_s = (int32_t*)(ws + p.off_tau);
    tau_p = (int32_t*)(ws + p.off_tau + qa);
    rerun = (int32_t*)(ws + p.off_tau + 2 * qa);
    qbflag = (int32_t*)(ws + p.off_tau + 3 * qa);
  }
};
int mfma_sample_select_launch(const MfmaPlan& p, const MfmaWorkspace& w, const uint8_t* q, int cb, int nq, int K,
                              hipStream_t s);
int mfma_sample_check_launch(const MfmaPlan& p, const MfmaWorkspace& w, int nq, int K, hipStream_t s);
int mfma_suffix_launch(const MfmaPlan& p, const MfmaWorkspace& w, const uint8_t* codes, int64_t n, int cb,
                       const uint8_t* q, int nq, int K, hipStream_t s);

constexpr int kMfmaKindRowsDim = 3;
int mfma_dim_min_queries(int cb);
int mfma_dim_plan(int64_t n, int cb, int nq, int K, MfmaPlan* p);
bool mfma_dim_use(int64_t n, int cb, int nq, int K, int flags);
int mfma_dim_scan_launch(const MfmaPlan& p, const uint8_t* codes, int64_t n, int cb, const uint8_t* q, int nq, int K,
                         uint8_t* ws, hipStream_t s, int flags);

constexpr int KMAX = 1024;
constexpr int MAX_LISTS = 4096;

struct Phase1Route {
  bool mfma;
  ScanPlan sp;
  MfmaPlan mp;
  size_t bytes;
  size_t off_lists;
  int nl;
  bool sorted;
};
int phase1_route(int64_t n, int cb, int nq, int K, int flags, Phase1Route* r);
int phase1_launch(const Phase1Route& r, const uint8_t* codes, int64_t n, int cb, const uint8_t* q, int nq, int K,
                  void* ws, hipStream_t s, int flags);
size_t phase1_workspace_bytes(int64_t n, int cb, int nq, int K);

constexpr int kLargeMaxChunks = 1024;
constexpr int64_t kLargeHistBytes = 64 << 20;
constexpr int kLargeQueryBatch = 512;

struct LargePlan {
  int qg;
  int nw;
  int64_t chunk_rows;
  int nchunks;
  size_t off_hist, off_prefix, off_tc, off_lists, off_s2, off_s3, off_ord, off_kp, bytes;
};
int large_plan(int64_t n, int cb, int nq, int K, LargePlan* p);
constexpr int kLargeStageCount = VRQ_LARGE_STAGE_COUNT, kLargeStageThreshold = VRQ_LARGE_STAGE_THRESHOLD,
              kLargeStageEmit = VRQ_LARGE_STAGE_EMIT,
              kLargeStageAll = kLargeStageCount | kLargeStageThreshold | kLargeStageEmit;
int large_scan_launch(const LargePlan& p, const uint8_t* codes, int64_t n, int cb, const uint8_t* q, int nq, int K,
                      uint8_t* ws, hipStream_t s, int stages, const uint64_t* allow = nullptr);
int64_t large_chunk_rows(int64_t n, int64_t want, int qb, int64_t bins);
void large_layout(LargePlan* p, int64_t n, int nq, int qb, int K, int64_t bins);
int large_threshold_launch(const uint32_t* hist, int nq, int nchunks, int bins, int want, int K, bool filtered,
                           int32_t* tc, int32_t* prefix, uint64_t* lists, hipStream_t s);

struct BatchPlan {
  int engine;
  LargePlan lp;
  int mb;
  int qpw;
  int nqb;
  int passes;
  int64_t flush_rows;
  size_t need;
};
int large_mfma_min_queries(int cb);
int batch_plan(int64_t n, int cb, int nq, int K, int engine, BatchPlan* p);
int batch_scan_launch(const BatchPlan& p, const uint8_t* codes, int64_t n, int cb, const uint8_t* q, int nq, int K,
                      uint8_t* ws, hipStream_t s, int stages, const uint64_t* allow);

}
```

Baseline: 37270 queries/s.

## Defer per-hit candidate emission to a separate expand kernel via block-level event queues

The MFMA Hamming scan no longer extracts individual hits, stages them in LDS and atomically appends them to per-query candidate lists inside the hot loop. It only records (block, lane-mask) events per wave into a small LDS ring and flushes them to a global queue. A new expand kernel then reloads the flagged 32-row blocks, recomputes exact Hamming distances with popcount and writes the per-query candidate lists and counts. This removes staging, atomics and flush work from the main scan. In exchange it adds an extra launch, re-reads the flagged rows, and can overflow when a queue's capacity is exceeded. In that case the count is set to capc+1, the same overflow marker the old path used.

```diff
diff --git a/vectorragquantization_amd/csrc/hamming_mfma.hip b/vectorragquantization_amd/csrc/hamming_mfma.hip
--- a/vectorragquantization_amd/csrc/hamming_mfma.hip
+++ b/vectorragquantization_amd/csrc/hamming_mfma.hip
@@ -17,6 +17,7 @@
 constexpr int GPW = (PKT / 1024) / MWAVES;
 constexpr int BAHEAD = 3;
 constexpr int NRING = BAHEAD < 4 ? 4 : 8;
+constexpr int EVR = 64;
 #ifndef VRQ_K1M_NSR
 #define VRQ_K1M_NSR 4
 #endif
@@ -29,9 +30,10 @@
   static constexpr int QPB = MWAVES * QPW;
   static constexpr int NSR = VRQ_K1M_NSR < MB ? VRQ_K1M_NSR : MB;
   static constexpr int SMEM =
-      NPK * PKT + NUB * UBT + NUB * RT * 4 + MWAVES * QPW * 8 + MWAVES * (STG + 1) * 4 + MWAVES * MB * 128;
+      NPK * PKT + NUB * UBT + NUB * RT * 4 + MWAVES * QPW * 4 + MWAVES * EVR * 16 + MWAVES * MB * 128;
   static_assert(SMEM <= 160 * 1024, "LDS budget");
 };
+static_assert(MWAVES == kK1mWaves, "the plan's event queues: one per wave");
 constexpr int kMbLarge = 4, kMbSmall = 2;
 constexpr int kMbLargeMinQueries = 512;
 constexpr int kRowsMaxQueries = 128;
@@ -44,8 +46,7 @@
 constexpr int k1m_pre(int g) { return ((g & 7) == 1 ? 1 : 0) + (g == 12 ? 2 : 0); }
 constexpr int k1m_post(int g, int mb, int nsr, bool dense) {
   const int j = g & 15;
-  return ((g & 7) == 6 ? 2 : 0) + (g == 28 ? 1 : 0) + (!dense && j >= 4 + mb + nsr && j < 4 + 2 * mb ? 4 : 0) +
-         (!dense && g == 20 + mb ? 1 : 0) + (!dense && g == 24 + mb ? 1 : 0);
+  return ((g & 7) == 6 ? 2 : 0) + (g == 28 ? 1 : 0) + (!dense && j >= 4 + mb + nsr && j < 4 + 2 * mb ? 4 : 0);
 }
 constexpr int k1m_wait(int gi, int mb, int nsr, bool dense) {
   const int g0 = gi - BAHEAD;
@@ -54,11 +55,25 @@
   return n < 15 ? n : 15;
 }
 
+__device__ __forceinline__ v4i* k1m_event_slot(v4i* evq, int qcap, int64_t qid, uint64_t* cand, int capc, int nchunks,
+                                               int chunk, int qbase, int s) {
+  if (evq) return evq + qid * qcap + s;
+  const int sh = 30 - __builtin_clz(capc);
+  return reinterpret_cast<v4i*>(cand + ((int64_t)(qbase + (s >> sh)) * nchunks + chunk) * capc) + (s & ((1 << sh) - 1));
+}
+__device__ __forceinline__ int k1m_queue_cap(const void* evq, int qcap, int nq, int qbase, int qpw, int capc) {
+  if (evq) return qcap;
+  int nl = nq - qbase;
+  nl = nl < 0 ? 0 : nl > qpw ? qpw : nl;
+  const int c = nl * (capc >> 1);
+  return c < qcap ? c : qcap;
+}
+
 template <int MODE, int MB>
 __global__ __launch_bounds__(MWAVES * 64, 1) void hamming_mfma_kernel(
     const uint8_t* __restrict__ codes, int64_t n, int64_t row_begin, const uint8_t* __restrict__ queries, int nq,
-    const int32_t* __restrict__ tau, uint64_t* __restrict__ cand, int32_t* __restrict__ ccnt, int capc,
-    int64_t chunk_rows, int64_t chunk_stride, int64_t tile_stride, int nchunks, int nqb,
+    const int32_t* __restrict__ tau, v4i* __restrict__ evq, int32_t* __restrict__ evn, int qcap,
+    uint64_t* __restrict__ cand, int capc, int64_t chunk_rows, int64_t chunk_stride, int64_t tile_stride, int nchunks, int nqb,
     const int32_t* __restrict__ rerun,
     const int32_t* __restrict__ qbflag, uint16_t* __restrict__ dv, int64_t dv_stride) {
   constexpr bool DENSE = MODE == MFMA_SAMPLE;
@@ -69,9 +84,8 @@
   uint8_t* ub = smem + NPK * PKT;
   int32_t* pcr = (int32_t*)(smem + NPK * PKT + NUB * UBT);
   const int w = __builtin_amdgcn_readfirstlane(threadIdx.x >> 6);
-  int32_t* lcnt = pcr + NUB * RT + w * QPW;
-  int32_t* tq = pcr + NUB * RT + MWAVES * QPW + w * QPW;
-  int32_t* stg = pcr + NUB * RT + 2 * MWAVES * QPW + w * (STG + 1);
+  int32_t* tq = pcr + NUB * RT + w * QPW;
+  int32_t* evr = pcr + NUB * RT + MWAVES * QPW + w * (EVR * 4);
 
   const int l = lane_id();
   const int h = l >> 5, ri = l & 31;
@@ -130,7 +144,7 @@
                                      16, 0, 0);
   };
   const uint32_t pk0 = lds_addr(pk), ub0 = lds_addr(ub), pcr0 = lds_addr(pcr);
-  const uint32_t lc0 = lds_addr(lcnt), stg0 = lds_addr(stg);
+  const uint32_t evr0 = lds_addr(evr);
   uint32_t usrc[4], udst[4];
 #pragma unroll
   for (int u = 0; u < 4; ++u) {
@@ -177,7 +191,7 @@
   for (int m = 0; m < MB; ++m)
 #pragma unroll
     for (int s = 0; s < KS; ++s) asm volatile("" : "+a"(A[m][s]));
-  float* sd = reinterpret_cast<float*>(pcr + NUB * RT + 2 * MWAVES * QPW + MWAVES * (STG + 1)) + w * MB * 32;
+  float* sd = reinterpret_cast<float*>(pcr + NUB * RT + MWAVES * QPW + MWAVES * EVR * 4) + w * MB * 32;
 #pragma unroll
   for (int m = 0; m < MB; ++m)
     if (l < 32) {
@@ -196,7 +210,6 @@
                                            5, 6, 7, 8, 9, 10, 11, 12, 13, 14, 15);
     a = __builtin_bit_cast(v16f, x);
   };
-  for (int i = l; i < QPW; i += 64) lcnt[i] = 0;
   __syncthreads();
   auto wait_tiles = [&](int k) __attribute__((always_inline)) {
     if (k <= 0) wait_vm<0>();
@@ -232,98 +245,31 @@
   wait_tiles(nissued - 3);
   wait_lgkm0();
 
-  const int64_t qstride = (int64_t)nchunks * capc;
-  uint64_t* const cbase = cand + ((int64_t)qbase * nchunks + chunk) * capc;
-  int nst = 0;
-  int fe = 0, fpos = 0, nfl = 0;
-  auto fkey = [&](int e, int64_t base_row) __attribute__((always_inline)) {
-    return ((uint64_t)(uint32_t)(e >> ENT_V_SHIFT) << KEY_ROW_BITS) | (uint64_t)(base_row + (e & 127));
-  };
-  auto store_flushed = [&](int t) __attribute__((always_inline)) {
-    if (__builtin_expect(nfl != 0, 0)) {
-      const int ql = (fe >> ENT_Q_SHIFT) & 127;
-#ifndef VRQ_K1M_PROBE_NOSTORE
-      if (l < nfl && fpos < capc) cbase[ql * qstride + fpos] = fkey(fe, row0 + (int64_t)(t - 2) * RT);
-#endif
-      nfl = 0;
-    }
-  };
-  auto flush_from = [&](int i_begin, int64_t base_row) __attribute__((always_inline)) {
-    int lf = l;
-    asm volatile("" : "+v"(lf));
-    if (nst > STG) {
-      for (int i = lf; i < QPW; i += 64) lds_add32(lc0 + (uint32_t)(i * 4), capc + 1);
-      nst = STG;
-    }
-    for (int i0 = i_begin; i0 < nst; i0 += 64) {
-      const int i = i0 + lf;
-      int e = 0, pos = 0;
-      if (i < nst) lds_read32(e, stg0 + (uint32_t)(i * 4));
-      asm volatile("s_waitcnt lgkmcnt(0)" : "+v"(e)::"memory");
-      const int ql = (e >> ENT_Q_SHIFT) & 127;
-      if (i < nst) lds_add_rtn32(pos, lc0 + (uint32_t)(ql * 4), 1);
-      asm volatile("s_waitcnt lgkmcnt(0)" : "+v"(pos)::"memory");
-      if (i < nst && pos < capc) cbase[ql * qstride + pos] = fkey(e, base_row);
-    }
-    nst = 0;
-  };
-  auto block_hits = [&](const v16f& a, int m, int pc, float hp, int rel7) __attribute__((always_inline)) {
-#pragma unroll
-    for (int g = 0; g < 16; ++g) {
-      const uint64_t mask = __ballot(a[g] > hp);
-      if (mask) {
-        int lo = l;
-        asm volatile("" : "+v"(lo));
-        if ((mask >> lo) & 1) {
-          const int below = __builtin_amdgcn_mbcnt_hi((uint32_t)(mask >> 32),
-                                                      __builtin_amdgcn_mbcnt_lo((uint32_t)mask, 0));
-          const int ql = 32 * m + (g & 3) + 8 * (g >> 2) + 4 * (lo >> 5);
-          const int v = pc - (int)(2.0f * a[g]);
-          const int pos = nst + below < STG ? nst + below : STG;
-          lds_write32(stg0 + (uint32_t)(pos * 4), ((v + ENT_V_BIAS) << ENT_V_SHIFT) | (ql << ENT_Q_SHIFT) | (rel7 - ri + (lo & 31)));
-        }
-        nst += __popcll(mask);
-      }
-    }
-  };
-  auto block_hits_fast = [&](const v16f& a, int m, int pc, float hp, int rel7) __attribute__((always_inline)) {
-    uint32_t m16 = 0, mmid = 0, mhi = 0;
-#pragma unroll
-    for (int g = 0; g < 7; ++g) m16 |= (a[g] > hp ? 1u : 0u) << g;
-    asm volatile("" : "+v"(m16));
-    VRQ_SCHED_FENCE();
-#pragma unroll
-    for (int g = 7; g < 14; ++g) mmid |= (a[g] > hp ? 1u : 0u) << (g - 7);
-    asm volatile("" : "+v"(mmid));
-    VRQ_SCHED_FENCE();
-#pragma unroll
-    for (int g = 14; g < 16; ++g) mhi |= (a[g] > hp ? 1u : 0u) << (g - 14);
-    asm volatile("" : "+v"(mmid), "+v"(mhi));
-    m16 |= (mmid << 7) | (mhi << 14);
-#ifdef VRQ_K1M_PROBE_NOSLOW
-    if (false) {
-#else
-    if (__ballot((m16 & (m16 - 1)) != 0)) {
-#endif
-      block_hits(a, m, pc, hp, rel7);
-    } else {
-      const uint64_t lanes = __ballot(m16 != 0);
-      if (m16) {
-        const v16i b = __builtin_bit_cast(v16i, a);
-        const int x0 = max(max(b[0], b[1]), b[2]), x1 = max(max(b[3], b[4]), b[5]), x2 = max(max(b[6], b[7]), b[8]);
-        const int x3 = max(max(b[9], b[10]), b[11]), x4 = max(max(b[12], b[13]), b[14]);
-        const float mx = __int_as_float(max(max(max(x0, x1), x2), max(max(x3, x4), b[15])));
-        const int below = __builtin_amdgcn_mbcnt_hi((uint32_t)(lanes >> 32),
-                                                    __builtin_amdgcn_mbcnt_lo((uint32_t)lanes, 0));
-        int lo = l;
-        asm volatile("" : "+v"(lo));
-        const int g = __builtin_ctz(m16);
-        const int ql = 32 * m + (g & 3) + 8 * (g >> 2) + 4 * (lo >> 5);
-        const int v = pc - (int)(2.0f * mx);
-        const int pos = nst + below < STG ? nst + below : STG;
-        lds_write32(stg0 + (uint32_t)(pos * 4), ((v + ENT_V_BIAS) << ENT_V_SHIFT) | (ql << ENT_Q_SHIFT) | (rel7 - ri + (lo & 31)));
-      }
-      nst += __popcll(lanes);
+  const int64_t qid = (int64_t)L * MWAVES + w;
+  const int wcap = DENSE ? 0 : k1m_queue_cap(evq, qcap, nq, qbase, QPW, capc);
+  uint64_t ah0 = 0, ah1 = 0;
+  int nev = 0, nfl = 0;
+  auto put_event = [&](int blk, uint64_t mask) __attribute__((always_inline)) {
+    int lo = l;
+    asm volatile("" : "+v"(lo));
+    const v4i e = {blk, (int)(uint32_t)mask, (int)(uint32_t)(mask >> 32), 0};
+    if (lo == 0) lds_write128(evr0 + (uint32_t)((nev & (EVR - 1)) * 16), e);
+    ++nev;
+  };
+  auto flush_events = [&](int cnt) __attribute__((always_inline)) {
+    int lo = l;
+    asm volatile("" : "+v"(lo));
+    v4i e;
+    lds_read128(e, evr0 + (uint32_t)(((nfl + lo) & (EVR - 1)) * 16));
+    asm volatile("s_waitcnt lgkmcnt(0)" : "+v"(e)::"memory");
+    if (lo < cnt && nfl + lo < wcap) *k1m_event_slot(evq, qcap, qid, cand, capc, nchunks, chunk, qbase, nfl + lo) = e;
+    nfl += cnt;
+  };
+  auto record = [&](int t) __attribute__((always_inline)) {
+    if (__builtin_expect((ah0 | ah1) != 0, 0)) {
+      if (ah0) put_event(2 * t - 3, ah0);
+      if (ah1) put_event(2 * t - 2, ah1);
+      if (nev - nfl >= EVR / 2) flush_events(EVR / 2);
     }
   };
   auto row_pc = [&](int pcv, int lr) __attribute__((always_inline)) {
@@ -338,7 +284,6 @@
   const uint32_t bl0 = ub0 + (uint32_t)(l * 16);
   int pcvP = 0;
   int lmax = 0;
-  uint64_t anyhit = 0;
   int hpb = 0;
   v16f acc[2][MB];
   v16f seedr[NSR > 0 ? NSR : 1];
@@ -381,7 +326,7 @@
   uint32_t st_a = 0, st_b = 0, st_bsum = 0;
 #endif
   for (int t = 0; t < ntiles; ++t) {
-    store_flushed(t);
+    if constexpr (!DENSE) record(t);
     const bool steady = t < nsteady;
     if (__builtin_expect(steady, 1)) {
       if constexpr (!VRQ_K1M_DMA_SHADOW) {
@@ -415,8 +360,8 @@
         lds_read128(pa, xor_add<0>(psrc0, pks));
         lds_read128(pb, xor_add<16>(psrc0, pks));
       }
-      asm volatile("s_waitcnt lgkmcnt(%7)"
-                   : "+v"(ring[gi & (NRING - 1)]), "+v"(pv), "+v"(pcv[0]), "+v"(pcv[1]), "+v"(pa), "+v"(pb), "+v"(fe)
+      asm volatile("s_waitcnt lgkmcnt(%6)"
+                   : "+v"(ring[gi & (NRING - 1)]), "+v"(pv), "+v"(pcv[0]), "+v"(pcv[1]), "+v"(pa), "+v"(pb)
                    : "n"(k1m_wait(gi, MB, NSR, DENSE))
                    : "memory");
       constexpr bool TEST = !DENSE && j >= 2 && j < 2 + MB;
@@ -446,7 +391,7 @@
           } else {
             const int mx = max(max(e3, e4), f0);
             lmax = tm == 0 ? max(bb[15], mx) : max(max(lmax, bb[15]), mx);
-            if constexpr (tm == MB - 1) anyhit = __ballot(lmax > hpb);
+            if constexpr (tm == MB - 1) (nbk == 0 ? ah0 : ah1) = __ballot(lmax > hpb);
           }
         }
         if constexpr (!DENSE && j == 1 && k == 0) {
@@ -523,29 +468,6 @@
             asm volatile("" : "+s"(dsrc));
           }
         }
-        if constexpr (k == 3) {
-          if constexpr (gi == 20 + MB && !DENSE) {
-            lds_read32(fe, stg0 + (uint32_t)(l * 4));
-            nfl = nst < 64 ? nst : 64;
-          }
-          if constexpr (gi == 24 + MB && !DENSE)
-            lds_add_rtn32(fpos, lc0 + (uint32_t)(((fe >> ENT_Q_SHIFT) & 127) * 4), l < nfl ? 1 : 0);
-          if constexpr (!DENSE && j == 3 + MB) {
-            if (__builtin_expect(anyhit != 0, 0)) {
-              const int pcr_ = nbk == 0 ? pcvP : pcv[0];
-              const int lr = (nbk == 0 ? (t - 1) * RT + 32 : t * RT) + ri;
-              const int pc = row_pc(pcr_, lr);
-              const float hp = 0.5f * (float)pc;
-              static_for<0, MB>([&](auto M) {
-                constexpr int mm = decltype(M)::value;
-#ifndef VRQ_K1M_PROBE_NOHITS
-                if (any_above(acc[nbk ^ 1][mm], hp))
-                  block_hits_fast(acc[nbk ^ 1][mm], mm, pc, hp, (nbk == 0 ? 32 : 64) + ri);
-#endif
-              });
-            }
-          }
-        }
       };
       static_for<0, MB>([&](auto M) {
         constexpr int m = decltype(M)::value;
@@ -585,31 +507,35 @@
       }
 #endif
     }
-    asm volatile("s_waitcnt lgkmcnt(0)" : "+v"(fpos), "+v"(fe)::"memory");
+    wait_lgkm0();
 #ifdef VRQ_K1M_STAMPS
     if (t > 0) st_bsum += st_b - st_a;
     st_a = st_an;
 #endif
-    if (__builtin_expect(nst > 64, 0))
-      flush_from(64, row0 + (int64_t)(t - 1) * RT);
-    nst = 0;
 #ifndef VRQ_K1M_PROBE_NOBARRIER
     barrier_all();
 #endif
   }
-  store_flushed(ntiles);
+  if constexpr (!DENSE) record(ntiles);
   if (ntiles > 0) {
     const int lr = (ntiles - 1) * RT + 32 + ri;
-    const int pc = row_pc(pcvP, lr);
-    const float hp = 0.5f * (float)pc;
-    static_for<0, MB>([&](auto M) {
-      constexpr int m = decltype(M)::value;
-      if constexpr (DENSE)
+    if constexpr (DENSE) {
+      static_for<0, MB>([&](auto M) {
+        constexpr int m = decltype(M)::value;
         block_dense(acc[1][m], m, pcvP, lr);
-      else
-        if (any_above(acc[1][m], hp)) block_hits_fast(acc[1][m], m, pc, hp, 96 + ri);
-    });
-    if (nst) flush_from(0, row0 + (int64_t)(ntiles - 2) * RT);
+      });
+    } else {
+      int mx = 0;
+      static_for<0, MB>([&](auto M) {
+        constexpr int m = decltype(M)::value;
+        const v16i bb = __builtin_bit_cast(v16i, acc[1][m]);
+#pragma unroll
+        for (int g = 0; g < 16; ++g) mx = max(mx, bb[g]);
+      });
+      const uint64_t last = __ballot(mx > __float_as_int(0.5f * (float)row_pc(pcvP, lr)));
+      if (last) put_event(2 * ntiles - 1, last);
+      if (nev != nfl) flush_events(nev - nfl);
+    }
   }
   wait_lgkm0();
 #ifdef VRQ_K1M_STAMPS
@@ -627,11 +553,141 @@
   else {
     int lz = l;
     asm volatile("" : "+v"(lz));
-    for (int i = lz; i < QPW; i += 64) {
-      const int q = qbase + i;
-      if (q < nq && (!rerun || rerun[q])) ccnt[(int64_t)q * nchunks + chunk] = lcnt[i];
-    }
-  }
+    if (lz == 0) evn[(int64_t)L * MWAVES + w] = nev;
+  }
+}
+
+template <int MODE, int MB>
+__global__ __launch_bounds__(2 * MWAVES * 64) void k1m_expand_kernel(
+    const uint8_t* __restrict__ codes, int64_t n, const uint8_t* __restrict__ queries, int nq,
+    const int32_t* __restrict__ tau, uint64_t* cand, int32_t* __restrict__ ccnt, int capc,
+    int64_t chunk_rows, int nchunks, int nqb, const int32_t* __restrict__ rerun, const int32_t* __restrict__ qbflag,
+    const v4i* evq, const int32_t* __restrict__ evn, int qcap) {
+  constexpr int QPW = MfmaShape<MB>::QPW, QPB = MfmaShape<MB>::QPB;
+  const int chunk = blockIdx.x / nqb, qb = blockIdx.x - chunk * nqb;
+  if (qbflag && qbflag[qb] == 0) return;
+  const int64_t row0 = (int64_t)chunk * chunk_rows;
+  if (row0 >= n) return;
+  const int wv = __builtin_amdgcn_readfirstlane(threadIdx.x >> 6);
+  const int w = wv >> 1, h = wv & 1;
+  const int l = lane_id();
+  const int qbase = qb * QPB + w * QPW;
+  const int64_t qid = ((int64_t)chunk * nqb + qb) * MWAVES + w;
+  __shared__ v4i evs[MWAVES][kK1mQueueCap];
+  const int wcap = k1m_queue_cap(evq, qcap, nq, qbase, QPW, capc);
+  const int len = __builtin_amdgcn_readfirstlane(evn[qid]);
+  {
+    const int ncopy = len < wcap ? len : wcap;
+    for (int s = h * 64 + l; s < ncopy; s += 128)
+      evs[w][s] = *k1m_event_slot(const_cast<v4i*>(evq), qcap, qid, cand, capc, nchunks, chunk, qbase, s);
+  }
+  __syncthreads();
+  const int m = l >> 4, g = l & 15;
+  const int q = qbase + 32 * m + (g & 3) + 8 * (g >> 2) + 4 * h;
+  const bool live = m < MB && q < nq && (!rerun || rerun[q]);
+  if (__ballot(live) == 0) return;
+  int32_t* const cnt = ccnt + (int64_t)(live ? q : 0) * nchunks + chunk;
+  if (len > wcap) {
+    if (live) *cnt = capc + 1;
+    return;
+  }
+  uint64_t* const list = cand + ((int64_t)(live ? q : 0) * nchunks + chunk) * capc;
+  uint32_t qw[32];
+  {
+    const uint4* qp = reinterpret_cast<const uint4*>(queries + (int64_t)(live ? q : 0) * 128);
+#pragma unroll
+    for (int c = 0; c < 8; ++c) {
+      const uint4 v = qp[c];
+      qw[4 * c] = v.x, qw[4 * c + 1] = v.y, qw[4 * c + 2] = v.z, qw[4 * c + 3] = v.w;
+    }
+  }
+  const int tq = live ? tau[q] : -0x40000000;
+  const v4i* const queue = evs[w];
+
+  const int qlast = len > 0 ? len - 1 : 0;
+  auto load_raw = [&](int base) __attribute__((always_inline)) -> v4i {
+    const int i = base + l;
+    return queue[i < qlast ? i : qlast];
+  };
+  auto take = [&](const v4i& e, int base, int& blk, uint32_t& mask) __attribute__((always_inline)) {
+    blk = e.x;
+    mask = base + l < len ? (uint32_t)(h ? e.z : e.y) : 0u;
+  };
+  int gbase = 0, eblk;
+  uint32_t emask;
+  take(load_raw(0), 0, eblk, emask);
+  uint64_t pend = __ballot(emask != 0);
+  uint32_t rem = 0;
+  int cb = 0;
+  auto next_row = [&]() __attribute__((always_inline)) -> int {
+    while (rem == 0) {
+      while (pend == 0) {
+        if (gbase + 64 >= len) return -1;
+        gbase += 64;
+        take(load_raw(gbase), gbase, eblk, emask);
+        pend = __ballot(emask != 0);
+      }
+      const int e = __builtin_ctzll(pend);
+      pend &= pend - 1;
+      rem = (uint32_t)__builtin_amdgcn_readlane((int)emask, e);
+      cb = __builtin_amdgcn_readlane(eblk, e);
+    }
+    const int bit = __builtin_ctz(rem);
+    rem &= rem - 1;
+    return cb * 32 + bit;
+  };
+  auto fetch = [&](int& vrow, v4i& d) __attribute__((always_inline)) {
+    vrow = -1;
+#pragma unroll
+    for (int j = 0; j < 8; ++j) {
+      const int r = next_row();
+      if (r < 0) break;
+      vrow = (l >> 3) == j ? r : vrow;
+    }
+    const uint8_t* p = codes + (row0 + (vrow < 0 ? 0 : vrow)) * 128 + (l & 7) * 16;
+    asm volatile("global_load_dwordx4 %0, %1, off" : "+v"(d) : "v"(p) : "memory");
+  };
+  auto landed = [](v4i& d) __attribute__((always_inline)) { asm volatile("s_waitcnt vmcnt(1)" : "+v"(d)::"memory"); };
+  auto xpc = [](uint32_t a, uint32_t b, int c) __attribute__((always_inline)) -> int {
+    int r;
+    asm("v_bcnt_u32_b32 %0, %1, %2" : "=v"(r) : "v"(a ^ b), "v"(c));
+    return r;
+  };
+  int pos = 0;
+  auto consume = [&](int vrow, const v4i& d) __attribute__((always_inline)) -> bool {
+#pragma unroll 1
+    for (int j = 0; j < 8; ++j) {
+      const int r = __builtin_amdgcn_readlane(vrow, 8 * j);
+      if (r < 0) return false;
+      int d0 = -tq, d1 = 0;
+#pragma unroll
+      for (int p = 0; p < 8; ++p) {
+        d0 = xpc((uint32_t)__builtin_amdgcn_readlane(d.x, 8 * j + p), qw[4 * p], d0);
+        d1 = xpc((uint32_t)__builtin_amdgcn_readlane(d.y, 8 * j + p), qw[4 * p + 1], d1);
+        d0 = xpc((uint32_t)__builtin_amdgcn_readlane(d.z, 8 * j + p), qw[4 * p + 2], d0);
+        d1 = xpc((uint32_t)__builtin_amdgcn_readlane(d.w, 8 * j + p), qw[4 * p + 3], d1);
+      }
+      const int v = d0 + d1;
+      if (v < 0) {
+        if (pos < capc) list[pos] = ((uint64_t)(uint32_t)(v + ENT_V_BIAS) << KEY_ROW_BITS) | (uint64_t)(row0 + r);
+        ++pos;
+      }
+    }
+    return true;
+  };
+  int vra, vrb;
+  v4i da = {0, 0, 0, 0}, db = {0, 0, 0, 0};
+  fetch(vra, da);
+  for (;;) {
+    fetch(vrb, db);
+    landed(da);
+    if (!consume(vra, da) || __ballot(live && pos <= capc) == 0) break;
+    fetch(vra, da);
+    landed(db);
+    if (!consume(vrb, db) || __ballot(live && pos <= capc) == 0) break;
+  }
+  asm volatile("s_waitcnt vmcnt(0)" : "+v"(da), "+v"(db)::"memory");
+  if (live) *cnt = pos;
 }
 
 constexpr double kSwapMaxPairs = 4294967296.0;
@@ -1557,11 +1613,22 @@
       hipLaunchKernelGGL(kswap4, dim3(grid), dim3(4 * 64), 0, s, codes, n, (int64_t)0, q, nq, tau, cd, cc, p.capc,
                          crows, cstride, (int64_t)RT, nch, p.nqb, rr, qf, d, dstride);
     else if (p.mb == kMbLarge)
-      hipLaunchKernelGGL(kern4, dim3(grid), dim3(MWAVES * 64), 0, s, codes, n, (int64_t)0, q, nq, tau, cd, cc, p.capc,
-                         crows, cstride, (int64_t)RT, nch, p.nqb, rr, qf, d, dstride);
+      hipLaunchKernelGGL(kern4, dim3(grid), dim3(MWAVES * 64), 0, s, codes, n, (int64_t)0, q, nq, tau, rr ? (v4i*)w.evq : (v4i*)nullptr, w.evn,
+                         rr ? p.qcap_r : p.qcap, w.cand, p.capc, crows, cstride, (int64_t)RT, nch, p.nqb, rr, qf, d, dstride);
     else
-      hipLaunchKernelGGL(kern2, dim3(grid), dim3(MWAVES * 64), 0, s, codes, n, (int64_t)0, q, nq, tau, cd, cc, p.capc,
-                         crows, cstride, (int64_t)RT, nch, p.nqb, rr, qf, d, dstride);
+      hipLaunchKernelGGL(kern2, dim3(grid), dim3(MWAVES * 64), 0, s, codes, n, (int64_t)0, q, nq, tau, rr ? (v4i*)w.evq : (v4i*)nullptr, w.evn,
+                         rr ? p.qcap_r : p.qcap, w.cand, p.capc, crows, cstride, (int64_t)RT, nch, p.nqb, rr, qf, d, dstride);
+  };
+  auto expand = [&](auto kern4, auto kern2, const int32_t* tau, const int32_t* rr, const int32_t* qf) {
+    if (p.swap) return;
+    if (p.mb == kMbLarge)
+      hipLaunchKernelGGL(kern4, dim3(p.nchunks * p.nqb), dim3(2 * MWAVES * 64), 0, s, codes, n, q, nq, tau, w.cand, w.ccnt,
+                         p.capc, p.chunk_rows, p.nchunks, p.nqb, rr, qf, rr ? (const v4i*)w.evq : (const v4i*)nullptr, (const int32_t*)w.evn,
+                         rr ? p.qcap_r : p.qcap);
+    else
+      hipLaunchKernelGGL(kern2, dim3(p.nchunks * p.nqb), dim3(2 * MWAVES * 64), 0, s, codes, n, q, nq, tau, w.cand, w.ccnt,
+                         p.capc, p.chunk_rows, p.nchunks, p.nqb, rr, qf, rr ? (const v4i*)w.evq : (const v4i*)nullptr, (const int32_t*)w.evn,
+                         rr ? p.qcap_r : p.qcap);
   };
   auto rows_pass = [&](auto k1, auto k2, auto k4, const int32_t* tau, const int32_t* rr, const int32_t* qf,
                        int nch, int64_t crows, int64_t cstride, int64_t tstride, uint16_t* d, int64_t dstride) {
@@ -1586,7 +1653,7 @@
     if (rc != VRQ_OK) return rc;
   } else if (st & VRQ_SCAN_STAGE_PREFIX) {
     hipLaunchKernelGGL((hamming_mfma_kernel<MFMA_SAMPLE, kMbSmall>), dim3(p.sample_chunks * p.nqb_s), dim3(MWAVES * 64),
-                       0, s, codes, n, (int64_t)0, q, nq, none, (uint64_t*)nullptr, (int32_t*)nullptr, 0,
+                       0, s, codes, n, (int64_t)0, q, nq, none, (v4i*)nullptr, (int32_t*)nullptr, 0, (uint64_t*)nullptr, 0,
                        p.sample_chunk_rows, p.sample_stride, p.sample_tile_stride, p.sample_chunks, p.nqb_s, none,
                        none, w.dv, p.dvcols);
     VRQ_LAUNCH_CHECK();
@@ -1610,6 +1677,9 @@
          (const int32_t*)(sampled ? w.tau_s : w.tau_p), w.cand, w.ccnt, p.chunk_rows, p.chunk_rows, p.nchunks, none, none,
          mdv, (int64_t)0);
     VRQ_LAUNCH_CHECK();
+    expand(k1m_expand_kernel<MFMA_MAIN, kMbLarge>, k1m_expand_kernel<MFMA_MAIN, kMbSmall>,
+           (const int32_t*)(sampled ? w.tau_s : w.tau_p), none, none);
+    VRQ_LAUNCH_CHECK();
   }
   if ((st & VRQ_SCAN_STAGE_RECHECK) && sampled) {
     const int rc = mfma_sample_check_launch(p, w, nq, K, s);
@@ -1619,12 +1689,16 @@
                 hamming_mfma_rows_kernel<MFMA_RERUN, 4>, (const int32_t*)w.tau_p, (const int32_t*)w.rerun,
                 (const int32_t*)w.qbflag, p.nchunks, p.chunk_rows, p.chunk_rows, (int64_t)RT, (uint16_t*)nullptr,
                 (int64_t)0);
-    else
+    else {
       pass(hamming_mfma_swap_kernel<MFMA_RERUN, 2, 8>, hamming_mfma_swap_kernel<MFMA_RERUN, 4, 4>,
            hamming_mfma_kernel<MFMA_RERUN, kMbLarge>,
            hamming_mfma_kernel<MFMA_RERUN, kMbSmall>, p.nchunks * p.nqb,
            (const int32_t*)w.tau_p, w.cand, w.ccnt, p.chunk_rows, p.chunk_rows, p.nchunks, (const int32_t*)w.rerun,
            (const int32_t*)w.qbflag, (uint16_t*)nullptr, (int64_t)0);
+      VRQ_LAUNCH_CHECK();
+      expand(k1m_expand_kernel<MFMA_RERUN, kMbLarge>, k1m_expand_kernel<MFMA_RERUN, kMbSmall>, (const int32_t*)w.tau_p,
+             (const int32_t*)w.rerun, (const int32_t*)w.qbflag);
+    }
     VRQ_LAUNCH_CHECK();
   }
   if (st & VRQ_SCAN_STAGE_SUFFIX) return mfma_suffix_launch(p, w, codes, n, 128, q, nq, K, s);
diff --git a/vectorragquantization_amd/csrc/mfma_threshold.hip b/vectorragquantization_amd/csrc/mfma_threshold.hip
--- a/vectorragquantization_amd/csrc/mfma_threshold.hip
+++ b/vectorragquantization_amd/csrc/mfma_threshold.hip
@@ -413,6 +413,14 @@
   p->off_cnt = p->off_cand + al((size_t)nq * p->nchunks * p->capc * sizeof(uint64_t));
   p->off_tau = p->off_cnt + al((size_t)nq * p->nchunks * sizeof(int32_t));
   p->bytes = p->off_tau + 3 * al((size_t)nq * sizeof(int32_t)) + (size_t)p->nqb * sizeof(int32_t);
+  const bool k1m = !p->rows && !p->swap;
+  const int64_t nblk = (p->chunk_rows + 31) / 32;
+  p->qcap = !k1m ? 0 : nblk < kK1mQueueCap ? (int)nblk : kK1mQueueCap;
+  const size_t nqueues = k1m ? (size_t)p->nchunks * p->nqb * kK1mWaves : 0;
+  const size_t dvb = (size_t)nq * p->dvcols * sizeof(uint16_t);
+  p->off_evq = al(nqueues * sizeof(int32_t));
+  const size_t per = k1m && dvb > p->off_evq ? (dvb - p->off_evq) / (nqueues * 16) : 0;
+  p->qcap_r = per < (size_t)p->qcap ? (int)per : p->qcap;
 }
 
 int mfma_sample_select_launch(const MfmaPlan& p, const MfmaWorkspace& w, const uint8_t* q, int cb, int nq, int K,
diff --git a/vectorragquantization_amd/csrc/vrq_scan.h b/vectorragquantization_amd/csrc/vrq_scan.h
--- a/vectorragquantization_amd/csrc/vrq_scan.h
+++ b/vectorragquantization_amd/csrc/vrq_scan.h
@@ -58,7 +58,11 @@
   int64_t chunk_rows;
   int nchunks;
   size_t off_suffix, off_cand, off_cnt, off_tau, bytes;
+  int qcap, qcap_r;
+  size_t off_evq;
 };
+constexpr int kK1mQueueCap = 2048;
+constexpr int kK1mWaves = 4;
 
 int mfma_plan(int64_t n, int nq, int K, MfmaPlan* p);
 bool mfma_use(int64_t n, int nq, int K, int flags);
@@ -71,7 +75,11 @@
   uint16_t* dv;
   uint64_t *suffix, *cand;
   int32_t *ccnt, *tau_s, *tau_p, *rerun, *qbflag;
+  uint8_t* evq;
+  int32_t* evn;
   MfmaWorkspace(const MfmaPlan& p, uint8_t* ws, int nq) {
+    evq = ws + p.off_evq;
+    evn = (int32_t*)ws;
     const size_t qa = ((size_t)nq * sizeof(int32_t) + 255) & ~size_t(255);
     dv = (uint16_t*)ws;
     suffix = (uint64_t*)(ws + p.off_suffix);
```

Result: no change. 37120 queries/s (-0.4%).
